# ubc-vision/StableKeypoints

Measured on AMD Instinct MI355X. Metric: images/sec for token-optimization step (SD1.5, 512^2, K=10 kpts), higher is better.
Workload: dtype f32 (fp32 MFMA / VALU throughout; flash attention of the >= 1024-key self-attention layers: 3xbf16 operand split, fp32 accumulate, error <= the fp32 kernel's)

## Files before the change

include/skp.h:

```cpp
#ifndef SKP_H
#define SKP_H

#include <stdint.h>

#ifdef __cplusplus
extern "C" {
#endif

#define SKP_MAX_LAYERS 8
#define SKP_MAX_SUBJECTS 4

#define SKP_E_BADARG (-1)
#define SKP_E_RANGE  (-2)
#define SKP_E_LDS    (-3)

int skp_abi_version(void);

int skp_tune_set(const char* key, int value);
int skp_tune_get(const char* key);

int skp_gemm_nt_f32(const float* A, const float* B, float* C, int M, int N, int K, int Z0, int Z1,
                    int64_t sa0, int64_t sa1, int64_t sam, int64_t sak,
                    int64_t sb0, int64_t sb1, int64_t sbn, int64_t sbk,
                    int64_t sc0, int64_t sc1, int64_t scm, float alpha, void* stream);

int skp_qk_logits_f32(const float* q, const float* k, float* S, int B, int Bk, int H, int T, int s2,
                      int d, float scale, void* stream);

int skp_attn_map_fwd_f32(const float* const* S , const int* s ,
                         int L, int B, int H, int T, int R, float* M, float* lse, void* stream);

int skp_attn_map_fwd_ex_f32(const float* const* S , const int* s , int L, int B, int H,
                            int T, int R, float* M, float* lse_out, const float* lse_in, int ldt,
                            int64_t m_bstride, int mode, void* stream);

int64_t skp_attn_map_bwd_workspace(const int* s , int L, int B, int H, int T, int R);

int skp_attn_map_bwd_f32(const float* const* S , float* const* dS ,
                         const int* s , int L, int B, int H, int T, int R,
                         const float* dM, const float* lse, float* workspace, void* stream);

int skp_attn_map_fwd_wide_f32(const float* const* S , const int* s , int L, int B, int H, int T,
                              int R, float* M, float* lse, const int* tokrow, int n_rows, int ldt, void* stream);
int skp_attn_map_fwd_wide_ok(const int* s , int L, int T, int R);

int skp_attn_map_bwd_col_ok(const int* s , int L, int H, int T, int R, int K);
int64_t skp_attn_map_bwd_col_workspace(const int* s , int L, int B, int H, int T, int R, int K);
int skp_attn_map_bwd_col_f32(const float* const* S , float* const* dS , const int* s , int L,
                             int B, int H, int T, int R, const int64_t* sel, const float* G, int K, const float* lse,
                             void* workspace, int ldt, void* stream);

int64_t skp_attn_map_bwd_sparse_workspace(const int* s , int L, int B, int H, int T, int R, int K);
int skp_attn_map_bwd_sparse_f32(const float* const* S , float* const* dS , const int* s ,
                                int L, int B, int H, int T, int R, const int64_t* sel, const float* G, int K,
                                const float* lse, void* workspace, int ldt, void* stream);

int skp_unwarp_accumulate_f32(const float* M, const float* theta_inv, int n, int K, int R, int S, float* tot, float* num,
                              int finish, void* stream);

int skp_group_norm_coef_f32(const float* x, const float* off, const float* gamma, const float* beta, float* mean, float* rstd,
                            float* coef, const float* bs, int nblk, int pix, float* workspace, int N, int C, int G, int HW,
                            float eps, void* stream);
int skp_conv3x3_f4_gn_ok(int B, int Cin, int Cout, int H, int W);
int skp_conv3x3_f4_gn_f32(const void* x, const void* U, const void* bias, const void* residual, void* y, float* stats,
                          const float* coef, int B, int Cin, int Cout, int H, int W, void* stream);

int skp_conv3x3_f4r_ok(int B, int Cin, int Cout, int H, int W);
int skp_conv3x3_f4r_filter_f32(const void* w, void* R, int Cout, int Cin, int flip_transpose, void* stream);
int64_t skp_conv3x3_f4r_workspace(int B, int Cin, int Cout, int H, int W);
int skp_conv3x3_f4r_f32(const void* x, const void* R, const void* bias, const void* residual, void* y, void* workspace,
                        int B, int Cin, int Cout, int H, int W, void* stream);

int skp_cross_attn_fwd_f32(const float* q, const float* k, const float* v, float* out, float* lse,
                           int B, int Bk, int H, int N, int T, int d, float scale, void* stream);
int64_t skp_cross_attn_bwd_workspace(int B, int H, int N, int T, int d);
int skp_cross_attn_bwd_f32(const float* q, const float* k, const float* v, const float* out,
                           const float* dout, const float* lse, float* dq, float* dk, float* dv,
                           float* workspace, int B, int Bk, int H, int N, int T, int d, float scale,
                           void* stream);

int skp_attn_map_bwd_ex_f32(const float* const* S , float* const* dS , const int* s ,
                            int L, int B, int H, int T, int R, const float* dM, const float* lse,
                            float* workspace, float* dot_io, int ldt, int64_t m_bstride, int mode, void* stream);

int64_t skp_flash_attn_bwd_workspace(int B, int Bk, int H, int N, int Nk, int d);
int skp_flash_attn_fwd_f32(const float* q, const float* k, const float* v, float* out, float* lse,
                           int B, int Bk, int H, int N, int Nk, int d, float scale, void* stream);
int skp_flash_attn_bwd_f32(const float* q, const float* k, const float* v, const float* out, const float* dout,
                           const float* lse, float* dq, float* dk, float* dv, float* workspace,
                           int B, int Bk, int H, int N, int Nk, int d, float scale, void* stream);
int skp_flash_attn_bwd_ld_f32(const float* q, const float* k, const float* v, const float* out, const float* dout,
                              const float* lse, float* dq, float* dk, float* dv, float* workspace,
                              int B, int Bk, int H, int N, int Nk, int d, float scale, int ldg, void* stream);

int skp_flash_attn_fwd_split_ok(int B, int Bk, int H, int N, int Nk, int d);
int64_t skp_flash_attn_fwd_split_workspace(int B, int Bk, int H, int N, int Nk, int d);
int skp_flash_attn_fwd_split_f32(const float* q, const float* k, const float* v, float* out, float* lse, void* workspace,
                                 int B, int Bk, int H, int N, int Nk, int d, float scale, void* stream);
int skp_flash_attn_bwd_split_ok(int B, int Bk, int H, int N, int Nk, int d);
int64_t skp_flash_attn_bwd_split_workspace(int B, int Bk, int H, int N, int Nk, int d);
int skp_flash_attn_bwd_split_f32(const float* q, const float* k, const float* v, const float* out, const float* dout,
                                 const float* lse, float* dq, float* dk, float* dv, void* workspace, int B, int Bk, int H, int N,
                                 int Nk, int d, float scale, void* stream);
int skp_flash_attn_bwd_split_ld_f32(const float* q, const float* k, const float* v, const float* out, const float* dout,
                                    const float* lse, float* dq, float* dk, float* dv, void* workspace, int B, int Bk, int H,
                                    int N, int Nk, int d, float scale, int ldg, void* stream);

int skp_self_attn_fwd_f32(const float* q, const float* k, const float* v, float* out, float* lse,
                          int B, int H, int N, int d, float scale, void* stream);
int skp_self_attn_bwd_f32(const float* q, const float* k, const float* v, const float* out, const float* dout,
                          const float* lse, float* dq, float* dk, float* dv, float* workspace,
                          int B, int H, int N, int d, float scale, void* stream);

int skp_group_norm_fwd_f32(const float* x, const float* off, const float* gamma, const float* beta, float* y,
                           float* mean, float* rstd, float* workspace, int N, int C, int G, int HW, float eps,
                           int silu, void* stream);
int skp_group_norm_onepass_ok(int N, int C, int G, int HW);
int skp_group_norm_bwd_f32(const float* x, const float* off, const float* gamma, const float* beta,
                           const float* dy, const float* mean, const float* rstd, float* dx, float* workspace,
                           int N, int C, int G, int HW, float eps, int silu, void* stream);
int skp_group_norm_bwd_add_f32(const float* x, const float* off, const float* gamma, const float* beta,
                               const float* dy, const float* mean, const float* rstd, float* dx, const float* dadd,
                               float* workspace, int N, int C, int G, int HW, float eps, int silu, void* stream);

int skp_add_bias_residual_f32(const float* a, const float* b, const float* bias, float* out, int N, int C, int HW,
                              void* stream);

int skp_add_layer_norm_ok(int C);
int skp_add_layer_norm_fwd_f32(const float* d, const float* h, const float* gamma, const float* beta, float* x, float* n,
                               float* stat, int64_t rows, int C, float eps, void* stream);
int skp_add_layer_norm_bwd_f32(const float* dn, const float* dskip, const float* x, const float* stat, const float* gamma,
                               float* dx, int64_t rows, int C, void* stream);

int skp_conv3x3_filter_f32(const void* w, void* U, int Cout, int Cin, int flip_transpose, void* stream);
int64_t skp_conv3x3_workspace(int B, int Cin, int Cout, int H, int W, int variant);
int skp_conv3x3_f32(const void* x, const void* U, const void* bias, const void* residual, void* y, void* workspace,
                    int B, int Cin, int Cout, int H, int W, int variant, void* stream);

int skp_conv3x3_f4_filter_f32(const void* w, void* U, int Cout, int Cin, int flip_transpose, void* stream);
int64_t skp_conv3x3_f4_workspace(int B, int Cin, int Cout, int H, int W);
int skp_conv3x3_f4_f32(const void* x, const void* U, const void* bias, const void* residual, void* y, void* workspace,
                       int B, int Cin, int Cout, int H, int W, void* stream);

int skp_conv3x3_f4_stats_blocks(int B, int Cin, int Cout, int H, int W);
int skp_conv3x3_f4_stats_f32(const void* x, const void* U, const void* bias, const void* residual, void* y, float* stats,
                             int B, int Cin, int Cout, int H, int W, void* stream);
int skp_conv3x3_s2_stats_f32(const void* x, const void* U, const void* bias, void* y, float* stats, int B, int Cin, int Cout,
                             int H, int W, int pad, void* stream);
int skp_group_norm_fwd_blocks_f32(const float* x, const float* off, const float* gamma, const float* beta, float* y,
                                  float* mean, float* rstd, const float* bs, int nblk, int pix, int N, int C, int G, int HW,
                                  float eps, int silu, void* stream);

int skp_conv3x3_s2_filter_f32(const void* w, void* U, int Cout, int Cin, void* stream);
int skp_conv3x3_s2_f32(const void* x, const void* U, const void* bias, void* y, int B, int Cin, int Cout, int H, int W,
                       int pad, void* stream);
int64_t skp_conv3x3_s2_workspace(int B, int Cin, int Cout, int H, int W);
int skp_conv3x3_s2_ws_f32(const void* x, const void* U, const void* bias, void* y, void* workspace, int B, int Cin, int Cout,
                          int H, int W, int pad, void* stream);

int skp_conv3x3_small_f32(const void* x, const void* w, const void* bias, void* y, int B, int Cin, int Cout, int H, int W,
                          void* stream);
int skp_conv3x3_small_stats_blocks(int B, int Cin, int Cout, int H, int W);
int skp_conv3x3_small_stats_f32(const void* x, const void* w, const void* bias, void* y, float* stats, int B, int Cin, int Cout,
                                int H, int W, void* stream);

int skp_geglu_fwd_f32(const float* p, float* y, int64_t rows, int inner, void* stream);
int skp_geglu_bwd_f32(const float* p, const float* dy, float* dp, int64_t rows, int inner, void* stream);

int skp_nchw_to_tokens_f32(const float* x, float* y, int B, int C, int HW, void* stream);
int skp_tokens_to_nchw_f32(const float* t, const float* residual, float* y, int B, int C, int HW, void* stream);

int skp_token_stats_f32(const float* M, int T, int R, int num_subjects, float sigma, float eps,
                        int32_t* argmax, float* kl, float* entropy, void* stream);

int skp_select_tokens(const float* kl, const int32_t* argmax_t, int T, int R, int n_cand, int top_k,
                      int64_t* cand, int64_t* sel, void* stream);
int skp_select_tokens_batched(const float* kl, const int32_t* argmax_t, int n, int T, int R, int n_cand, int top_k,
                              int64_t* cand, int64_t* sel, void* stream);

int skp_losses_fwd_f32(const float* M, const float* Mt, const int64_t* sel, int K, int T, int R,
                       const int32_t* argmax, int num_subjects, float sigma,
                       const float* theta_inv , float* partial, float* g_sharp,
                       float* g_eq_a, float* g_eq_b, void* stream);
int skp_losses_fwd_dev_f32(const float* M, const float* Mt, const int64_t* sel, int K, int T, int R,
                           const int32_t* argmax, int num_subjects, float sigma, const float* theta_inv_dev,
                           float* partial, float* g_sharp, float* g_eq_a, float* g_eq_b, void* stream);

int skp_rows_axpy_f32(float* dst, const int64_t* sel, int K, int64_t n, const float* x, const float* a,
                      const float* y, const float* b, void* stream);

#ifdef __cplusplus
}
#endif
#endif
```

stablekeypoints_amd/_native.py:

```python
from __future__ import annotations

import ctypes as C
import os

import torch

_HERE = os.path.dirname(os.path.abspath(__file__))
LIB_PATH = os.environ.get("SKP_LIB_PATH") or os.path.join(_HERE, "csrc", "libskp_hip.so")
ABI_VERSION = 39

_vp, _i, _f, _i64 = C.c_void_p, C.c_int, C.c_float, C.c_int64

SIGNATURES = {
    "skp_abi_version": [],
    "skp_tune_set": [C.c_char_p, _i],
    "skp_tune_get": [C.c_char_p],
    "skp_group_norm_onepass_ok": [_i, _i, _i, _i],
    "skp_gemm_nt_f32": [_vp, _vp, _vp, _i, _i, _i, _i, _i,
                        _i64, _i64, _i64, _i64, _i64, _i64, _i64, _i64, _i64, _i64, _i64, _f, _vp],
    "skp_qk_logits_f32": [_vp, _vp, _vp, _i, _i, _i, _i, _i, _i, _f, _vp],
    "skp_attn_map_fwd_f32": [C.POINTER(_vp), C.POINTER(_i), _i, _i, _i, _i, _i, _vp, _vp, _vp],
    "skp_attn_map_fwd_ex_f32": [C.POINTER(_vp), C.POINTER(_i), _i, _i, _i, _i, _i, _vp, _vp, _vp, _i, _i64, _i, _vp],
    "skp_attn_map_bwd_ex_f32": [C.POINTER(_vp), C.POINTER(_vp), C.POINTER(_i), _i, _i, _i, _i, _i, _vp, _vp, _vp, _vp,
                                _i, _i64, _i, _vp],
    "skp_attn_map_bwd_workspace": [C.POINTER(_i), _i, _i, _i, _i, _i],
    "skp_attn_map_bwd_f32": [C.POINTER(_vp), C.POINTER(_vp), C.POINTER(_i), _i, _i, _i, _i, _i, _vp, _vp, _vp, _vp],
    "skp_group_norm_coef_f32": [_vp, _vp, _vp, _vp, _vp, _vp, _vp, _vp, _i, _i, _vp, _i, _i, _i, _i, _f, _vp],
    "skp_conv3x3_f4_gn_ok": [_i, _i, _i, _i, _i],
    "skp_conv3x3_f4_gn_f32": [_vp, _vp, _vp, _vp, _vp, _vp, _vp, _i, _i, _i, _i, _i, _vp],
    "skp_unwarp_accumulate_f32": [_vp, _vp, _i, _i, _i, _i, _vp, _vp, _i, _vp],
    "skp_attn_map_fwd_wide_f32": [C.POINTER(_vp), C.POINTER(_i), _i, _i, _i, _i, _i, _vp, _vp, _vp, _i, _i, _vp],
    "skp_attn_map_fwd_wide_ok": [C.POINTER(_i), _i, _i, _i],
    "skp_attn_map_bwd_col_ok": [C.POINTER(_i), _i, _i, _i, _i, _i],
    "skp_attn_map_bwd_col_workspace": [C.POINTER(_i), _i, _i, _i, _i, _i, _i],
    "skp_attn_map_bwd_col_f32": [C.POINTER(_vp), C.POINTER(_vp), C.POINTER(_i), _i, _i, _i, _i, _i, _vp, _vp, _i, _vp, _vp,
                                 _i, _vp],
    "skp_attn_map_bwd_sparse_workspace": [C.POINTER(_i), _i, _i, _i, _i, _i, _i],
    "skp_attn_map_bwd_sparse_f32": [C.POINTER(_vp), C.POINTER(_vp), C.POINTER(_i), _i, _i, _i, _i, _i, _vp, _vp, _i, _vp, _vp,
                                    _i, _vp],
    "skp_token_stats_f32": [_vp, _i, _i, _i, _f, _f, _vp, _vp, _vp, _vp],
    "skp_select_tokens": [_vp, _vp, _i, _i, _i, _i, _vp, _vp, _vp],
    "skp_select_tokens_batched": [_vp, _vp, _i, _i, _i, _i, _i, _vp, _vp, _vp],
    "skp_losses_fwd_f32": [_vp, _vp, _vp, _i, _i, _i, _vp, _i, _f, C.POINTER(_f), _vp, _vp, _vp, _vp, _vp],
    "skp_losses_fwd_dev_f32": [_vp, _vp, _vp, _i, _i, _i, _vp, _i, _f, _vp, _vp, _vp, _vp, _vp, _vp],
    "skp_rows_axpy_f32": [_vp, _vp, _i, _i64, _vp, _vp, _vp, _vp, _vp],
    "skp_cross_attn_fwd_f32": [_vp, _vp, _vp, _vp, _vp, _i, _i, _i, _i, _i, _i, _f, _vp],
    "skp_cross_attn_bwd_workspace": [_i, _i, _i, _i, _i],
    "skp_cross_attn_bwd_f32": [_vp, _vp, _vp, _vp, _vp, _vp, _vp, _vp, _vp, _vp, _i, _i, _i, _i, _i, _i, _f, _vp],
    "skp_group_norm_fwd_f32": [_vp, _vp, _vp, _vp, _vp, _vp, _vp, _vp, _i, _i, _i, _i, _f, _i, _vp],
    "skp_group_norm_bwd_f32": [_vp, _vp, _vp, _vp, _vp, _vp, _vp, _vp, _vp, _i, _i, _i, _i, _f, _i, _vp],
    "skp_group_norm_bwd_add_f32": [_vp, _vp, _vp, _vp, _vp, _vp, _vp, _vp, _vp, _vp, _i, _i, _i, _i, _f, _i, _vp],
    "skp_add_bias_residual_f32": [_vp, _vp, _vp, _vp, _i, _i, _i, _vp],
    "skp_add_layer_norm_ok": [_i],
    "skp_add_layer_norm_fwd_f32": [_vp, _vp, _vp, _vp, _vp, _vp, _vp, _i64, _i, _f, _vp],
    "skp_add_layer_norm_bwd_f32": [_vp, _vp, _vp, _vp, _vp, _vp, _i64, _i, _vp],
    "skp_conv3x3_filter_f32": [_vp, _vp, _i, _i, _i, _vp],
    "skp_conv3x3_workspace": [_i, _i, _i, _i, _i, _i],
    "skp_conv3x3_f32": [_vp, _vp, _vp, _vp, _vp, _vp, _i, _i, _i, _i, _i, _i, _vp],
    "skp_conv3x3_f4_filter_f32": [_vp, _vp, _i, _i, _i, _vp],
    "skp_conv3x3_f4_workspace": [_i, _i, _i, _i, _i],
    "skp_conv3x3_f4_f32": [_vp, _vp, _vp, _vp, _vp, _vp, _i, _i, _i, _i, _i, _vp],
    "skp_flash_attn_fwd_split_ok": [_i, _i, _i, _i, _i, _i],
    "skp_flash_attn_fwd_split_workspace": [_i, _i, _i, _i, _i, _i],
    "skp_flash_attn_fwd_split_f32": [_vp, _vp, _vp, _vp, _vp, _vp, _i, _i, _i, _i, _i, _i, C.c_float, _vp],
    "skp_flash_attn_bwd_split_ok": [_i, _i, _i, _i, _i, _i],
    "skp_flash_attn_bwd_split_workspace": [_i, _i, _i, _i, _i, _i],
    "skp_flash_attn_bwd_split_f32": [_vp, _vp, _vp, _vp, _vp, _vp, _vp, _vp, _vp, _vp, _i, _i, _i, _i, _i, _i, _f, _vp],
    "skp_flash_attn_bwd_split_ld_f32": [_vp, _vp, _vp, _vp, _vp, _vp, _vp, _vp, _vp, _vp, _i, _i, _i, _i, _i, _i, _f, _i, _vp],
    "skp_conv3x3_f4r_ok": [_i, _i, _i, _i, _i],
    "skp_conv3x3_f4r_filter_f32": [_vp, _vp, _i, _i, _i, _vp],
    "skp_conv3x3_f4r_workspace": [_i, _i, _i, _i, _i],
    "skp_conv3x3_f4r_f32": [_vp, _vp, _vp, _vp, _vp, _vp, _i, _i, _i, _i, _i, _vp],
    "skp_conv3x3_s2_filter_f32": [_vp, _vp, _i, _i, _vp],
    "skp_conv3x3_s2_f32": [_vp, _vp, _vp, _vp, _i, _i, _i, _i, _i, _i, _vp],
    "skp_conv3x3_s2_workspace": [_i, _i, _i, _i, _i],
    "skp_conv3x3_s2_ws_f32": [_vp, _vp, _vp, _vp, _vp, _i, _i, _i, _i, _i, _i, _vp],
    "skp_conv3x3_small_f32": [_vp, _vp, _vp, _vp, _i, _i, _i, _i, _i, _vp],
    "skp_conv3x3_small_stats_blocks": [_i, _i, _i, _i, _i],
    "skp_conv3x3_small_stats_f32": [_vp, _vp, _vp, _vp, _vp, _i, _i, _i, _i, _i, _vp],
    "skp_conv3x3_f4_stats_blocks": [_i, _i, _i, _i, _i],
    "skp_conv3x3_f4_stats_f32": [_vp, _vp, _vp, _vp, _vp, _vp, _i, _i, _i, _i, _i, _vp],
    "skp_conv3x3_s2_stats_f32": [_vp, _vp, _vp, _vp, _vp, _i, _i, _i, _i, _i, _i, _vp],
    "skp_group_norm_fwd_blocks_f32": [_vp, _vp, _vp, _vp, _vp, _vp, _vp, _vp, _i, _i, _i, _i, _i, _i, _f, _i, _vp],
    "skp_geglu_fwd_f32": [_vp, _vp, _i64, _i, _vp],
    "skp_geglu_bwd_f32": [_vp, _vp, _vp, _i64, _i, _vp],
    "skp_nchw_to_tokens_f32": [_vp, _vp, _i, _i, _i, _vp],
    "skp_tokens_to_nchw_f32": [_vp, _vp, _vp, _i, _i, _i, _vp],
    "skp_flash_attn_fwd_f32": [_vp, _vp, _vp, _vp, _vp, _i, _i, _i, _i, _i, _i, _f, _vp],
    "skp_flash_attn_bwd_workspace": [_i, _i, _i, _i, _i, _i],
    "skp_flash_attn_bwd_f32": [_vp, _vp, _vp, _vp, _vp, _vp, _vp, _vp, _vp, _vp, _i, _i, _i, _i, _i, _i, _f, _vp],
    "skp_flash_attn_bwd_ld_f32": [_vp, _vp, _vp, _vp, _vp, _vp, _vp, _vp, _vp, _vp, _i, _i, _i, _i, _i, _i, _f, _i, _vp],
    "skp_self_attn_fwd_f32": [_vp, _vp, _vp, _vp, _vp, _i, _i, _i, _i, _f, _vp],
    "skp_self_attn_bwd_f32": [_vp, _vp, _vp, _vp, _vp, _vp, _vp, _vp, _vp, _vp, _i, _i, _i, _i, _f, _vp],
}

_ERR = {-1: "SKP_E_BADARG (null pointer / non-positive size)",
        -2: "SKP_E_RANGE (size outside the built kernel range)",
        -3: "SKP_E_LDS (tile exceeds 160 KiB LDS)"}

_lib = None


class NativeLibraryError(RuntimeError):
    pass


def lib():
    global _lib
    if _lib is not None:
        return _lib
    if not os.path.exists(LIB_PATH):
        raise NativeLibraryError(
            f"{LIB_PATH} is missing: build it with `python -c 'import __graft_entry__ as g; g.build()'` "
            "(or `make -C stablekeypoints_amd/csrc`). There is no CPU/eager fallback for the hot path.")
    l = C.CDLL(LIB_PATH)
    for name, argtypes in SIGNATURES.items():
        if not hasattr(l, name):
            raise NativeLibraryError(f"{LIB_PATH} does not export {name}")
        fn = getattr(l, name)
        fn.argtypes = argtypes
        fn.restype = C.c_int64 if name.endswith("_workspace") else C.c_int
    v = l.skp_abi_version()
    if v != ABI_VERSION:
        raise NativeLibraryError(f"ABI mismatch: library {v}, binding {ABI_VERSION}")
    _lib = l
    return l


LAB_PATH = os.environ.get("SKP_LAB_PATH") or os.path.join(os.path.dirname(_HERE), "tools", "csrc", "libskp_lab.so")
LAB_SIGNATURES = {
    "skp_probe_mfma_f32": [_i, _i, _vp, _vp, _vp],
}
_lab = None


def lab():
    global _lab
    if _lab is None:
        if not os.path.exists(LAB_PATH):
            raise NativeLibraryError(f"{LAB_PATH} is missing: `make -C tools/csrc` (measurement aids, not the product library)")
        l = C.CDLL(LAB_PATH)
        for name, argtypes in LAB_SIGNATURES.items():
            fn = getattr(l, name)
            fn.argtypes, fn.restype = argtypes, C.c_int
        _lab = l
    return _lab


def check(rc: int, what: str):
    if rc == 0:
        return
    if rc < 0:
        raise RuntimeError(f"{what}: {_ERR.get(rc, rc)}")
    raise RuntimeError(f"{what}: HIP launch failed with hipError_t={rc}")


def ptr_array(ptrs):
    arr = (C.c_void_p * len(ptrs))(*[C.c_void_p(int(p)) for p in ptrs])
    return C.cast(arr, C.POINTER(C.c_void_p)), arr


def int_array(vals):
    arr = (C.c_int * len(vals))(*[int(v) for v in vals])
    return C.cast(arr, C.POINTER(C.c_int)), arr


def float_array(vals):
    arr = (C.c_float * len(vals))(*[float(v) for v in vals])
    return C.cast(arr, C.POINTER(C.c_float)), arr


def tune(key: str, value: int) -> None:
    check(lib().skp_tune_set(key.encode(), int(value)), f"skp_tune_set({key})")
```

stablekeypoints_amd/csrc/skp_conv_wino4.hip:

```cpp
#include <algorithm>
#include <type_traits>
#include "skp_common.h"
#include "skp_wino4_common.h"
#include <stdlib.h>

namespace {

__global__ void skp_wino4_filter_kernel(const float* __restrict__ w, float* __restrict__ U, int Cout, int Cin, int flip_t) {
    const int idx = blockIdx.x * blockDim.x + threadIdx.x;
    if (idx >= Cout * Cin) return;
    const int co = idx / Cin, ci = idx - co * Cin;
    float g[3][3];
    if (!flip_t) {
        const float* p = w + ((size_t)co * Cin + ci) * 9;
#pragma unroll
        for (int a = 0; a < 3; ++a)
#pragma unroll
            for (int b = 0; b < 3; ++b) g[a][b] = p[a * 3 + b];
    } else {
        const float* p = w + ((size_t)ci * Cout + co) * 9;
#pragma unroll
        for (int a = 0; a < 3; ++a)
#pragma unroll
            for (int b = 0; b < 3; ++b) g[a][b] = p[(2 - a) * 3 + (2 - b)];
// ... 113 lines not shown
#pragma unroll
    for (int tb = 0; tb < 2; ++tb) {
        const int tg = tile0 + tb * 16 + i16;
        t_ok[tb] = tg < a.nTiles;
        const int tgc = t_ok[tb] ? tg : 0;
        const int b = tgc / a.tilesPerImg, rem = tgc - b * a.tilesPerImg;
        const int ty = rem / a.tilesX, tx = rem - ty * a.tilesX;
        o_base[tb] = ((b * a.Cout) * a.H + 4 * ty) * a.W + 4 * tx;
    }

#pragma unroll
    for (int i = 0; i < 6; ++i) { load_row(cin_begin, 0, i); load_row(cin_begin, 1, i); }
#pragma unroll
    for (int k = 0; k < 3; ++k) { col_pass(0, k); col_pass(1, k); }
#pragma unroll
    for (int i = 0; i < 6; ++i) row_pass_store(0, i);
    f32x4 ua[W4_RING];
#pragma unroll
    for (int q = 0; q < W4_RING - 1; ++q) ua[q] = skp_buf_load_f32x4(urs, uvo, (cin_begin >> 4) * u_c16 + q * u_p, 0);
    __syncthreads();

    auto run_stage = [&](int s, auto mode_c) {
        constexpr int MODE = decltype(mode_c)::value;
        const f32x4* vb = vst + (s & 1) * W4_STAGE_F4 + kq * 32 + i16;
        const int ub = ((cin_begin >> 4) + s) * u_c16;
        f32x4 va[3][2];
        va[0][0] = vb[0];
        va[0][1] = vb[16];
        va[1][0] = vb[128];
        va[1][1] = vb[128 + 16];
        w4_unroll([&](auto pc) {
            constexpr int p = decltype(pc)::value;
            {
                constexpr int D = W4_RING - 1;
                constexpr int q = p + D;
                if (MODE == 0 || q < 36) {
                    const int uo = q < 36 ? ub + q * u_p : ub + u_c16 + (q - 36) * u_p;
                    ua[q % W4_RING] = skp_buf_load_f32x4(urs, uvo, uo, 0);
                }
            }
            if (MODE == 0) {
                if (p < 6) {
                    load_row(cin_begin + (s + 1) * 16, 0, p);
                    load_row(cin_begin + (s + 1) * 16, 1, p);
                } else if (p >= 24 && p < 30) {
                    col_pass((p - 24) & 1, (p - 24) >> 1);
                } else if (p >= 30) {
                    row_pass_store((s + 1) & 1, p - 30);
                }
            }
            if (p + 2 < 36) {
                va[(p + 2) % 3][0] = vb[(p + 2) * 128];
                va[(p + 2) % 3][1] = vb[(p + 2) * 128 + 16];
            }
            w4_unroll([&](auto mc) {
                constexpr int m = decltype(mc)::value;
                w4c_mfma<p, 0>(accv, ua[p % W4_RING][m], va[p % 3][0][m]);
                w4c_mfma<p, 1>(accv, ua[p % W4_RING][m], va[p % 3][1][m]);
            }, std::make_integer_sequence<int, 4>{});
            __builtin_amdgcn_sched_barrier(0);
        }, std::make_integer_sequence<int, 36>{});
    };
    for (int s = 0; s + 1 < nsteps; ++s) {
        run_stage(s, std::integral_constant<int, 0>{});
        __syncthreads();
    }
    run_stage(nsteps - 1, std::integral_constant<int, 1>{});
    if (STATS) __syncthreads();

    const i32x4 yrs = skp_make_rsrc(a.y + zsplit * a.y_split_stride, a.y_bytes);
    const i32x4 rrs = skp_make_rsrc(a.res, a.res ? a.y_bytes : 0u);
    const i32x4 brs = skp_make_rsrc(a.bias, a.bias ? (unsigned)a.Cout * 4u : 0u);
    f32x4 rr[4][2][4];
    float bvs[4];
    auto load_res = [&](int r) {
        const int co = n0 + 4 * kq + r;
#pragma unroll
        for (int tb = 0; tb < 2; ++tb) {
            const bool ok = t_ok[tb] && co < a.Cout;
            const int vo = (o_base[tb] + co * HW) * 4;
#pragma unroll
            for (int oy = 0; oy < 4; ++oy) rr[r][tb][oy] = skp_buf_load_f32x4(rrs, ok ? vo + oy * a.W * 4 : SKP_OOB, 0, 0);
        }
    };
#pragma unroll
    for (int r = 0; r < 4; ++r) {
        const int co = n0 + 4 * kq + r;
        bvs[r] = skp_buf_load_f32(brs, co < a.Cout ? co * 4 : SKP_OOB, 0, 0);
    }
    load_res(0);
    load_res(1);
    asm volatile("s_nop 15\n\ts_nop 15" ::: "memory");
    __builtin_amdgcn_sched_barrier(0);
    w4_unroll([&](auto rc) {
        constexpr int r = decltype(rc)::value;
        const int co = n0 + 4 * kq + r;
        const float bv = bvs[r];
        if (r + 2 < 4) load_res(r + 2);
        w4_unroll([&](auto tbc) {
            constexpr int tb = decltype(tbc)::value;
            const bool ok = t_ok[tb] && co < a.Cout;
            const int vo = (o_base[tb] + co * HW) * 4;
            float t[6][4];
            w4_unroll([&](auto ic) {
                constexpr int i = decltype(ic)::value;
                float m[6];
                w4_unroll([&](auto jc) { constexpr int j = decltype(jc)::value; m[j] = w4c_acc<i * 6 + j, tb, r>(accv); },
                          std::make_integer_sequence<int, 6>{});
                w4_out1d(m, t[i]);
            }, std::make_integer_sequence<int, 6>{});
#pragma unroll
            for (int ox = 0; ox < 4; ++ox) {
                float m[6], yv[4];
#pragma unroll
                for (int i = 0; i < 6; ++i) m[i] = t[i][ox];
                w4_out1d(m, yv);
#pragma unroll
                for (int oy = 0; oy < 4; ++oy) rr[r][tb][oy][ox] += yv[oy] + bv;
            }
#pragma unroll
            for (int oy = 0; oy < 4; ++oy) skp_buf_store_f32x4(rr[r][tb][oy], yrs, ok ? vo + oy * a.W * 4 : SKP_OOB, 0, 0);
            if (STATS) w4_park_stats((f32x2*)vst, wave * 8 + r * 2 + tb, lane, rr[r][tb], ok);
            __builtin_amdgcn_sched_barrier(0);
        }, std::make_integer_sequence<int, 2>{});
    }, std::make_integer_sequence<int, 4>{});
    if (STATS) {
        __syncthreads();
        if (tid < 128) {
            const int wv = tid >> 5, tb = (tid >> 4) & 1, lc = tid & 15;
            w4_store_stats(a, (const f32x2*)vst, wv * 8 + (lc & 3) * 2 + tb, lc >> 2, tile0 + tb * 16, (cg * 4 + wv) * 16 + lc);
        }
    }
}

__global__ void skp_wino4r_filter_kernel(const float* __restrict__ w, float* __restrict__ R, int Cout, int Cin, int flip_t) {
    const int idx = blockIdx.x * blockDim.x + threadIdx.x;
    if (idx >= Cout * Cin) return;
    const int co = idx / Cin, ci = idx - co * Cin;
    const int c16 = ci >> 4, kq = (ci >> 2) & 3, m = ci & 3, cb = co >> 4, i16 = co & 15, CB = Cout >> 4;
    float* dst = R + ((size_t)(c16 * CB + cb) * 9 * 64 + kq * 16 + i16) * 4 + m;
#pragma unroll
    for (int t = 0; t < 9; ++t) {
        const float v = flip_t ? w[((size_t)ci * Cout + co) * 9 + (8 - t)] : w[((size_t)co * Cin + ci) * 9 + t];
        dst[t * 256] = v;
    }
}

__global__ __launch_bounds__(256) void skp_wino4r_input_kernel(const float* __restrict__ x, float* __restrict__ Vg, int B, int Cin, int H,
                                                               int W, int tilesX, int tilesPerImg, int nTiles, int vpad) {
    const int idx = blockIdx.x * 256 + threadIdx.x;
    const int m = idx & 3, rest = idx >> 2;
    const int tg = rest % vpad, q4 = rest / vpad;
    if (q4 >= (Cin >> 2)) return;
    const bool tv = tg < nTiles;
    const int tgc = tv ? tg : 0;
    const int b = tgc / tilesPerImg, rem = tgc - b * tilesPerImg;
    const int ty = rem / tilesX, tx = rem - ty * tilesX;
    const float dsc[6] = {0.25f, -1.f / 6, -1.f / 6, 1.f / 24, 1.f / 24, 1.f};
    const float* xc = x + ((size_t)b * Cin + q4 * 4 + m) * H * W;
    float d[6][6];
#pragma unroll
    for (int i = 0; i < 6; ++i) {
        const int r = 4 * ty - 1 + i;
        const bool rv = tv && r >= 0 && r < H;
        const float* row = xc + r * W + 4 * tx;
        const f32x4 mid = rv ? *(const f32x4*)row : f32x4{0.f, 0.f, 0.f, 0.f};
        d[i][0] = (rv && tx > 0) ? row[-1] : 0.f;
        d[i][1] = mid[0]; d[i][2] = mid[1]; d[i][3] = mid[2]; d[i][4] = mid[3];
        d[i][5] = (rv && tx + 1 < tilesX) ? row[4] : 0.f;
    }
#pragma unroll
    for (int j = 0; j < 6; ++j) {
        float v[6], t[6];
#pragma unroll
        for (int i = 0; i < 6; ++i) v[i] = d[i][j];
        w4_in1d(v, t);
#pragma unroll
        for (int i = 0; i < 6; ++i) d[i][j] = t[i];
    }
    const int c16 = q4 >> 2, kq = q4 & 3;
    float* dst = Vg + (((size_t)c16 * 36 * 4 + kq) * vpad + tg) * 4 + m;
#pragma unroll
    for (int i = 0; i < 6; ++i) {
        float t[6];
        w4_in1d(d[i], t);
#pragma unroll
        for (int j = 0; j < 6; ++j) dst[(size_t)(i * 6 + j) * 16 * vpad] = t[j] * (dsc[i] * dsc[j]);
    }
}

#ifdef W4R_STAMPS
__device__ unsigned long long w4r_stamps[2][64];
#define W4R_STAMP(k) do { if (tid == 0 && (blockIdx.x == 0 || blockIdx.x == 100) && (k) < 64) w4r_stamps[blockIdx.x ? 1 : 0][k] = __builtin_readcyclecounter(); } while (0)
#else
#define W4R_STAMP(k) do { } while (0)
#endif
template <bool PART, int NTB = 2>
__global__ __launch_bounds__(256, 1) void skp_wino4r_conv_kernel(Wino4Args a) {
    extern __shared__ f32x4 vst[];
    const int tid = threadIdx.x, lane = tid & 63, wave = __builtin_amdgcn_readfirstlane(tid >> 6);
    const int i16 = lane & 15, kq = lane >> 4;
    int tblock, cg, zsplit;
    if (!w4_work(a, blockIdx.x + blockIdx.z * gridDim.x, tblock, cg, zsplit)) return;
    W4R_STAMP(0);
    const int tile0 = tblock * 32;
    const int n0 = (cg * 4 + wave) * 16;
    const int HW = a.H * a.W;
    const int nsteps = min(a.steps, a.total_steps - zsplit * a.steps);
    const int c16_0 = zsplit * a.steps;
    const i32x4 vrs = skp_make_rsrc(a.x, a.x_bytes);
    const i32x4 wrs = skp_make_rsrc(a.U, a.u_bytes);

    const int v_vo = ((tid >> 5) * a.vpad + tile0 + (tid & 31)) * 16;
    const int v_row8 = a.vpad * 128;
    auto load_v = [&](int c16, int buf, int r) {
        skp_buf_load_lds(vrs, (skp_lds_ptr)(vst + buf * W4_STAGE_F4 + r * 256 + wave * 64), 16, v_vo, c16 * 18 * v_row8 + r * v_row8, 0, 0);
    };
    const int CB = a.Cout >> 4;
    const int w_cb = ((cg * 4 + wave) * 9) * 1024;
    const int w_c16 = CB * 9 * 1024;
    f32x4 g[9], gn[9];
    auto load_g = [&](f32x4 (&dst)[9], int c16) {
#pragma unroll
        for (int t = 0; t < 9; ++t) dst[t] = skp_buf_load_f32x4(wrs, lane * 16, c16 * w_c16 + w_cb + t * 1024, 0);
    };
    f32x4 ut[3];
    auto u_piece = [&](const f32x4 (&gg)[9], int i, int piece, f32x4 (&u)[6]) {
        if (piece < 3) {
            const int b = piece;
            const f32x4 g0 = gg[b], g1 = gg[3 + b], g2 = gg[6 + b];
            ut[b] = i == 0 ? g0 : i == 5 ? g2 : i == 1 ? (g0 + g2) + g1 : i == 2 ? (g0 + g2) - g1
                  : i == 3 ? (g0 + 4.f * g2) + 2.f * g1 : (g0 + 4.f * g2) - 2.f * g1;
        } else if (piece == 3) {
            const f32x4 s2 = ut[0] + ut[2];
            u[0] = ut[0]; u[5] = ut[2];
            u[1] = s2 + ut[1]; u[2] = s2 - ut[1];
        } else if (piece == 4) {
            const f32x4 e = ut[0] + 4.f * ut[2];
            u[3] = e + 2.f * ut[1];
        } else {
            const f32x4 e = ut[0] + 4.f * ut[2];
            u[4] = e - 2.f * ut[1];
        }
    };
    auto u_row = [&](const f32x4 (&gg)[9], int i, f32x4 (&u)[6]) {
#pragma unroll
        for (int k = 0; k < 6; ++k) u_piece(gg, i, k, u);
    };

    w4_unroll([&](auto rc) { asm volatile("v_accvgpr_write_b32 a[%0], 0" : : "n"(decltype(rc)::value) : W4_AGPR_CLOBBERS); },
              std::make_integer_sequence<int, 256>{});
    f32x4 accv[4][2];
#pragma unroll
    for (int p = 0; p < 4; ++p)
#pragma unroll
        for (int tb = 0; tb < 2; ++tb) accv[p][tb] = f32x4{0.f, 0.f, 0.f, 0.f};

    int o_base[2];
    bool t_ok[2];
#pragma unroll
    for (int tb = 0; tb < 2; ++tb) {
        const int tg = tile0 + tb * 16 + i16;
        t_ok[tb] = tg < a.nTiles;
        const int tgc = t_ok[tb] ? tg : 0;
        const int b = tgc / a.tilesPerImg, rem = tgc - b * a.tilesPerImg;
        const int ty = rem / a.tilesX, tx = rem - ty * a.tilesX;
        o_base[tb] = ((b * a.Cout) * a.H + 4 * ty) * a.W + 4 * tx;
    }

#pragma unroll
    for (int r = 0; r < 18; ++r) load_v(c16_0, 0, r);
    load_g(g, c16_0);
    f32x4 ur[2][6];
    u_row(g, 0, ur[0]);
    asm volatile("s_waitcnt vmcnt(0)" ::: "memory");
    __syncthreads();
    W4R_STAMP(1);

    for (int s = 0; s < nsteps; ++s) {
        const f32x4* vb = vst + (s & 1) * W4_STAGE_F4 + kq * 32 + i16;
        const int c16n = c16_0 + min(s + 1, nsteps - 1);
        f32x4 va[3][2];
        va[0][0] = vb[0];
        va[1][0] = vb[128];
        if (NTB == 2) { va[0][1] = vb[16]; va[1][1] = vb[128 + 16]; }
        w4_unroll([&](auto pc) {
            constexpr int p = decltype(pc)::value, i = p / 6, j = p - 6 * i;
            if (p == 0) load_g(gn, c16n);
            else if (p <= 18) load_v(c16n, (s + 1) & 1, p - 1);
            if (i < 5) u_piece(g, i + 1, j, ur[(i + 1) & 1]);
            if (p + 2 < 36) {
                va[(p + 2) % 3][0] = vb[(p + 2) * 128];
                if (NTB == 2) va[(p + 2) % 3][1] = vb[(p + 2) * 128 + 16];
            }
            w4_unroll([&](auto mc) {
                constexpr int m = decltype(mc)::value;
                w4c_mfma<p, 0>(accv, ur[i & 1][j][m], va[p % 3][0][m]);
                if constexpr (NTB == 2) w4c_mfma<p, 1>(accv, ur[i & 1][j][m], va[p % 3][1][m]);
            }, std::make_integer_sequence<int, 4>{});
            __builtin_amdgcn_sched_barrier(0);
        }, std::make_integer_sequence<int, 36>{});
#pragma unroll
        for (int t = 0; t < 9; ++t) g[t] = gn[t];
        u_row(g, 0, ur[0]);
        asm volatile("s_waitcnt vmcnt(0)" ::: "memory");
        __syncthreads();
        W4R_STAMP(2 + s);
    }

    asm volatile("s_nop 15\n\ts_nop 15" ::: "memory");
    __builtin_amdgcn_sched_barrier(0);
    const i32x4 yrs = skp_make_rsrc(a.y + zsplit * a.y_split_stride, a.y_bytes);
    if (PART) {
        w4_unroll([&](auto rc) {
            constexpr int r = decltype(rc)::value;
            const int co = n0 + 4 * kq + r;
            w4_unroll([&](auto tbc) {
                constexpr int tb = decltype(tbc)::value;
                const bool ok = t_ok[tb] && co < a.Cout;
                const int vo = (o_base[tb] + co * HW) * 4;
                float t[6][4];
                w4_unroll([&](auto ic) {
                    constexpr int i = decltype(ic)::value;
                    float m[6];
                    w4_unroll([&](auto jc) { constexpr int j = decltype(jc)::value; m[j] = w4c_acc<i * 6 + j, tb, r>(accv); },
                              std::make_integer_sequence<int, 6>{});
                    w4_out1d(m, t[i]);
                }, std::make_integer_sequence<int, 6>{});
                f32x4 o[4];
#pragma unroll
                for (int ox = 0; ox < 4; ++ox) {
                    float m[6], yv[4];
#pragma unroll
                    for (int i = 0; i < 6; ++i) m[i] = t[i][ox];
                    w4_out1d(m, yv);
#pragma unroll
                    for (int oy = 0; oy < 4; ++oy) o[oy][ox] = yv[oy];
                }
#pragma unroll
                for (int oy = 0; oy < 4; ++oy) skp_buf_store_f32x4(o[oy], yrs, ok ? vo + oy * a.W * 4 : SKP_OOB, 0, 0);
                __builtin_amdgcn_sched_barrier(0);
// ... 297 lines not shown
                w4_unroll([&](auto jc) { constexpr int j = decltype(jc)::value; m[j] = w4c_acc<i * 6 + j, cb, r>(accv); },
                          std::make_integer_sequence<int, 6>{});
                w4_out1d(m, t[i]);
            }, std::make_integer_sequence<int, 6>{});
#pragma unroll
            for (int ox = 0; ox < 4; ++ox) {
                float m[6], yv[4];
#pragma unroll
                for (int i = 0; i < 6; ++i) m[i] = t[i][ox];
                w4_out1d(m, yv);
#pragma unroll
                for (int oy = 0; oy < 4; ++oy) rr[e][oy][ox] += yv[oy] + bv;
            }
#pragma unroll
            for (int oy = 0; oy < 4; ++oy) skp_buf_store_f32x4(rr[e][oy], yrs, ok ? vo + oy * a.W * 4 : SKP_OOB, 0, 0);
            if (STATS) w4_park_stats(sst, wave * 8 + e, lane, rr[e], ok);
            __builtin_amdgcn_sched_barrier(0);
        }, std::make_integer_sequence<int, 8>{});
        if (STATS) {
            __syncthreads();
            if (tid < 128) {
                const int wv = tid >> 5, lc = tid & 31;
                w4_store_stats(a, sst, wv * 8 + ((lc >> 4) << 2) + (lc & 3), (lc >> 2) & 3, tile0, (cg * 4 + wv) * 32 + lc);
            }
        }
        if (!has_next) break;
        bpar = (bpar + nsteps) & 1;
        wid = wnext; tblock = tb_n; cg = cg_n; zsplit = z_n;
    }
}

static bool wino4_use_c128(int Cout, int tiles) {
    return tiles >= 128 && (Cout % 128 == 0 || (Cout > 128 && Cout % 128 >= 64));
}

static Wino4Grid wino4_grid(int Cout, int tiles, int S) {
    Wino4Grid g;
    const bool c128 = wino4_use_c128(Cout, tiles);
    g.ntb = c128 ? (tiles + 15) / 16 : (tiles + 31) / 32;
    g.ncg = c128 ? (Cout + 127) / 128 : (Cout + 63) / 64;
    g.tb_per_xcd = g.ntb >= (c128 ? 64 : 32) ? (g.ntb + 7) / 8 : 0;
    if (g.tb_per_xcd) {
        g.gx = 8u * g.tb_per_xcd * g.ncg;
        g.rounds = (int)((g.gx * (unsigned)S + 255) / 256);
    } else {
        const int upx = (g.ncg * S + 7) / 8;
        g.gx = 8u * upx * g.ntb;
        g.rounds = (upx * g.ntb + 31) / 32;
    }
    return g;
}

int wino4_plan(int B, int Cin, int Cout, int H, int W) {
    if (B <= 0 || Cin <= 0 || Cout <= 0 || H <= 0 || W <= 0) return 0;
    if ((Cin % 16) || (Cout % 16) || (H % 4) || (W % 4)) return 0;
    const int tiles = B * (H / 4) * (W / 4);
    const bool c128 = wino4_use_c128(Cout, tiles);
    const int nsteps = Cin / 16;
    const double out_bytes = (double)B * Cout * H * W * 4;
    if (const int S = skp_tune(SKP_TUNE_WINO_SPLIT)) {
        if (S >= 1 && S <= 16 && (S - 1) * ((nsteps + S - 1) / S) < nsteps) return S;
    }
    int best = 1;
    double best_cost = 1e30;
    const bool ragged_c128 = c128 && (Cout % 128) != 0;
    const double stage_us = c128 ? (ragged_c128 ? 4.8 : 3.9) : 5.6;
    for (int S = 1; S <= 16; ++S) {
        const int per = (nsteps + S - 1) / S;
        if ((S - 1) * per >= nsteps) continue;
        const Wino4Grid g = wino4_grid(Cout, tiles, S);
        double cost = g.rounds * (per + 2.0) * stage_us;
        if (S > 1) cost += 6.0 + (S + 1) * out_bytes / 8.0e6;
        if (cost < best_cost * (S > 1 ? (ragged_c128 ? 0.95 : 0.92) : 1.0)) { best_cost = cost; best = S; }
    }
    return best;
}

static Wino4Grid wino4r_grid(int Cout, int tiles, int S) {
    Wino4Grid g;
    g.ntb = (tiles + 31) / 32;
    g.ncg = Cout / 64;
    g.tb_per_xcd = g.ntb >= 32 ? (g.ntb + 7) / 8 : 0;
    if (g.tb_per_xcd) {
        g.gx = 8u * g.tb_per_xcd * g.ncg;
        g.rounds = (int)((g.gx * (unsigned)S + 255) / 256);
    } else {
        const int upx = (g.ncg * S + 7) / 8;
        g.gx = 8u * upx * g.ntb;
        g.rounds = (upx * g.ntb + 31) / 32;
    }
    return g;
}
static int wino4r_max_tiles() { return skp_tune(SKP_TUNE_WINO_RAW_MAX_TILES); }
static bool wino4r_layout_ok(int B, int Cin, int Cout, int H, int W) {
    if (B <= 0 || Cin <= 0 || Cout <= 0 || H <= 0 || W <= 0) return false;
    if ((Cin % 16) || (Cout % 64) || (H % 4) || (W % 4)) return false;
    const long long tiles = (long long)B * (H / 4) * (W / 4);
    const long long vpad = (tiles + 31) / 32 * 32;
    return 36ll * Cin * vpad * 4 < 0x7fffffffll && 9ll * Cin * Cout * 4 < 0x7fffffffll && (long long)B * Cout * H * W * 4 < 0x7fffffffll;
}
static bool wino4r_shape_ok(int B, int Cin, int Cout, int H, int W) {
    if (!wino4r_layout_ok(B, Cin, Cout, H, W)) return false;
    const long long tiles = (long long)B * (H / 4) * (W / 4);
    if (wino4r_max_tiles() > 0) return tiles <= wino4r_max_tiles() && Cin >= 256;
    if (Cin >= 1280 && Cout >= 1280) return tiles <= 1536;
    return tiles <= 512 && (Cin >= 1920 || Cout >= 1920) && Cin >= 640 && Cout >= 640;
}
constexpr double W4R_STAGE1_US = 2.7;
static int wino4r_plan(int B, int Cin, int Cout, int H, int W) {
    const int tiles = B * (H / 4) * (W / 4);
    const int nsteps = Cin / 16;
    const double out_bytes = (double)B * Cout * H * W * 4;
    if (const int S = skp_tune(SKP_TUNE_WINO_SPLIT)) {
        if (S >= 1 && S <= 16 && (S - 1) * ((nsteps + S - 1) / S) < nsteps) return S;
    }
    int best = 1;
    double best_cost = 1e30;
    const double stage_us = tiles <= 16 ? W4R_STAGE1_US : 4.8, over = tiles <= 16 ? 2.0 : 2.5;
    for (int S = 1; S <= 16; ++S) {
        const int per = (nsteps + S - 1) / S;
        if ((S - 1) * per >= nsteps) continue;
        const Wino4Grid g = wino4r_grid(Cout, tiles, S);
        double cost = g.rounds * (per + over) * stage_us;
        if (S > 1) cost += 6.0 + (S + 1) * out_bytes / 8.0e6;
        if (cost < best_cost * (S > 1 ? 0.97 : 1.0)) { best_cost = cost; best = S; }
    }
    return best;
}

}

extern "C" int skp_conv3x3_f4_filter_f32(const void* w, void* U, int Cout, int Cin, int flip_transpose, void* stream) {
    if (!w || !U || Cout <= 0 || Cin <= 0) return SKP_E_BADARG;
    if (Cin & 15) return SKP_E_RANGE;
    const int n = Cout * Cin;
    hipLaunchKernelGGL(skp_wino4_filter_kernel, dim3((n + 255) / 256), dim3(256), 0, (hipStream_t)stream, (const float*)w,
                       (float*)U, Cout, Cin, flip_transpose);
    return skp_launch_status();
}

extern "C" int64_t skp_conv3x3_f4_workspace(int B, int Cin, int Cout, int H, int W) {
    const int S = wino4_plan(B, Cin, Cout, H, W);
    return S > 1 ? (int64_t)S * B * Cout * H * W * (int64_t)sizeof(float) : 0;
}

extern "C" int skp_conv3x3_f4_stats_blocks(int B, int Cin, int Cout, int H, int W) {
    const int S = wino4_plan(B, Cin, Cout, H, W);
    if (S != 1) return 0;
    const int tpi = (H / 4) * (W / 4);
    return (tpi % 32 == 0) ? tpi / 16 : 0;
}

static int wino4_run(const void* x, const void* U, const void* bias, const void* residual, void* y, void* workspace, float* stats,
                     int B, int Cin, int Cout, int H, int W, void* stream, const float* gncoef = nullptr);

extern "C" int skp_conv3x3_f4_gn_ok(int B, int Cin, int Cout, int H, int W) {
    if (wino4_plan(B, Cin, Cout, H, W) != 1) return 0;
    const int tiles = B * (H / 4) * (W / 4);
    const int max_cout = skp_tune(SKP_TUNE_GN_FOLD_MAX_COUT) ? skp_tune(SKP_TUNE_GN_FOLD_MAX_COUT) : 512;
    return (wino4_use_c128(Cout, tiles) && Cout <= max_cout) ? 1 : 0;
}

extern "C" int skp_conv3x3_f4_gn_f32(const void* x, const void* U, const void* bias, const void* residual, void* y,
                                     float* stats, const float* coef, int B, int Cin, int Cout, int H, int W, void* stream) {
    if (!coef) return SKP_E_BADARG;
    if (!skp_conv3x3_f4_gn_ok(B, Cin, Cout, H, W)) return SKP_E_RANGE;
    if (stats && skp_conv3x3_f4_stats_blocks(B, Cin, Cout, H, W) == 0) return SKP_E_RANGE;
    return wino4_run(x, U, bias, residual, y, nullptr, stats, B, Cin, Cout, H, W, stream, coef);
}

extern "C" int skp_conv3x3_f4_f32(const void* x, const void* U, const void* bias, const void* residual, void* y,
                                  void* workspace, int B, int Cin, int Cout, int H, int W, void* stream) {
    return wino4_run(x, U, bias, residual, y, workspace, nullptr, B, Cin, Cout, H, W, stream);
}

extern "C" int skp_conv3x3_f4_stats_f32(const void* x, const void* U, const void* bias, const void* residual, void* y,
                                        float* stats, int B, int Cin, int Cout, int H, int W, void* stream) {
    if (!stats || skp_conv3x3_f4_stats_blocks(B, Cin, Cout, H, W) == 0) return SKP_E_RANGE;
    return wino4_run(x, U, bias, residual, y, nullptr, stats, B, Cin, Cout, H, W, stream);
}

static int wino4_run(const void* x, const void* U, const void* bias, const void* residual, void* y, void* workspace, float* stats,
                     int B, int Cin, int Cout, int H, int W, void* stream, const float* gncoef) {
    if (!x || !U || !y) return SKP_E_BADARG;
    int S = wino4_plan(B, Cin, Cout, H, W);
    if (S == 0) return (B <= 0 || Cin <= 0 || Cout <= 0 || H <= 0 || W <= 0) ? SKP_E_BADARG : SKP_E_RANGE;
    if (!workspace) S = 1;
    const unsigned long long xb = (unsigned long long)B * Cin * H * W * 4, ub = (unsigned long long)36 * Cin * Cout * 4,
                             yb = (unsigned long long)B * Cout * H * W * 4;
    if (xb >= 0x80000000ull || ub >= 0x80000000ull || yb >= 0x80000000ull) return SKP_E_RANGE;
    Wino4Args a;
    a.x = (const float*)x; a.U = (const float*)U;
    a.B = B; a.Cin = Cin; a.Cout = Cout; a.H = H; a.W = W;
    a.tilesX = W / 4;
    a.tilesPerImg = a.tilesX * (H / 4);
    a.nTiles = B * a.tilesPerImg;
    a.x_bytes = (unsigned)xb; a.u_bytes = (unsigned)ub; a.y_bytes = (unsigned)yb;
    a.total_steps = Cin / 16;
    a.steps = (a.total_steps + S - 1) / S;
    a.splits = S;
    const size_t out_elems = (size_t)B * Cout * H * W;
    a.y_split_stride = out_elems;
    a.y = S > 1 ? (float*)workspace : (float*)y;
    a.bias = S > 1 ? nullptr : (const float*)bias;
    a.res = S > 1 ? nullptr : (const float*)residual;
    a.stats = S > 1 ? nullptr : stats;
    a.sblk = a.tilesPerImg / 16;
    a.gncoef = gncoef;
    hipStream_t st = (hipStream_t)stream;
    const size_t lds = (size_t)2 * W4_STAGE_F4 * sizeof(f32x4), lds_c = (size_t)2 * W4C_STAGE_F4 * sizeof(f32x4) + 32 * 64 * sizeof(f32x2);
    static bool attr_set = false;
    if (!attr_set) {
        hipError_t e = hipFuncSetAttribute((const void*)skp_wino4_conv_kernel<false>, hipFuncAttributeMaxDynamicSharedMemorySize, (int)lds);
        if (e != hipSuccess) return (int)e;
        e = hipFuncSetAttribute((const void*)skp_wino4_conv_kernel<true>, hipFuncAttributeMaxDynamicSharedMemorySize, (int)lds);
        if (e != hipSuccess) return (int)e;
        e = hipFuncSetAttribute((const void*)skp_wino4_conv_c128_kernel<false>, hipFuncAttributeMaxDynamicSharedMemorySize, (int)lds_c);
        if (e != hipSuccess) return (int)e;
        e = hipFuncSetAttribute((const void*)skp_wino4_conv_c128_kernel<true>, hipFuncAttributeMaxDynamicSharedMemorySize, (int)lds_c);
        if (e != hipSuccess) return (int)e;
        e = hipFuncSetAttribute((const void*)skp_wino4_conv_c128_kernel<true, true>, hipFuncAttributeMaxDynamicSharedMemorySize, (int)lds_c);
        if (e != hipSuccess) return (int)e;
        e = hipFuncSetAttribute((const void*)skp_wino4_conv_c128_kernel<false, true>, hipFuncAttributeMaxDynamicSharedMemorySize, (int)lds_c);
        if (e != hipSuccess) return (int)e;
        attr_set = true;
    }
    const bool c128 = wino4_use_c128(Cout, a.nTiles);
    const Wino4Grid g = wino4_grid(Cout, a.nTiles, S);
    a.ntb = g.ntb; a.ncg = g.ncg; a.tb_per_xcd = g.tb_per_xcd;
    a.gx = (int)g.gx;
    a.vtotal = g.tb_per_xcd ? (int)g.gx * S : (int)g.gx;
    static const int persist = [] {
        int dev = 0, ncu = 0;
        if (hipGetDevice(&dev) != hipSuccess || hipDeviceGetAttribute(&ncu, hipDeviceAttributeMultiprocessorCount, dev) != hipSuccess) ncu = 256;
        return ncu;
    }();
    const dim3 grid = c128 ? dim3((unsigned)(persist >= 8 ? std::min(a.vtotal, persist & ~7) : a.vtotal), 1, 1)
                           : (g.tb_per_xcd ? dim3(g.gx, 1, S) : dim3(g.gx, 1, 1));
    if (c128) {
        if (gncoef) {
            if (a.stats) hipLaunchKernelGGL((skp_wino4_conv_c128_kernel<true, true>), grid, dim3(256), lds_c, st, a);
            else hipLaunchKernelGGL((skp_wino4_conv_c128_kernel<false, true>), grid, dim3(256), lds_c, st, a);
        } else if (a.stats) hipLaunchKernelGGL((skp_wino4_conv_c128_kernel<true>), grid, dim3(256), lds_c, st, a);
        else hipLaunchKernelGGL((skp_wino4_conv_c128_kernel<false>), grid, dim3(256), lds_c, st, a);
    } else if (gncoef) {
        return SKP_E_RANGE;
    } else {
        if (a.stats) hipLaunchKernelGGL(skp_wino4_conv_kernel<true>, grid, dim3(256), lds, st, a);
        else hipLaunchKernelGGL(skp_wino4_conv_kernel<false>, grid, dim3(256), lds, st, a);
    }
    int rc = skp_launch_status();
    if (rc || S == 1) return rc;
    const size_t n4 = out_elems / 4;
    hipLaunchKernelGGL(skp_wino4_reduce_kernel, dim3((unsigned)((n4 + 255) / 256)), dim3(256), 0, st, (const float*)workspace,
                       (const float*)bias, (const float*)residual, (float*)y, n4, out_elems, S, (H * W) / 4, Cout);
    return skp_launch_status();
}

extern "C" int skp_conv3x3_f4r_ok(int B, int Cin, int Cout, int H, int W) {
    return wino4r_shape_ok(B, Cin, Cout, H, W) ? 1 : 0;
}

extern "C" int skp_conv3x3_f4r_filter_f32(const void* w, void* R, int Cout, int Cin, int flip_transpose, void* stream) {
    if (!w || !R || Cout <= 0 || Cin <= 0) return SKP_E_BADARG;
    if ((Cin & 15) || (Cout & 15)) return SKP_E_RANGE;
    const int n = Cout * Cin;
    hipLaunchKernelGGL(skp_wino4r_filter_kernel, dim3((n + 255) / 256), dim3(256), 0, (hipStream_t)stream, (const float*)w,
                       (float*)R, Cout, Cin, flip_transpose);
    return skp_launch_status();
}

extern "C" int64_t skp_conv3x3_f4r_workspace(int B, int Cin, int Cout, int H, int W) {
    if (!wino4r_layout_ok(B, Cin, Cout, H, W)) return 0;
    const int64_t tiles = (int64_t)B * (H / 4) * (W / 4), vpad = (tiles + 31) / 32 * 32;
    const int S = wino4r_plan(B, Cin, Cout, H, W);
    return 36 * (int64_t)Cin * vpad * 4 + (S > 1 ? (int64_t)S * B * Cout * H * W * 4 : 0);
}

extern "C" int skp_conv3x3_f4r_f32(const void* x, const void* R, const void* bias, const void* residual, void* y, void* workspace,
                                   int B, int Cin, int Cout, int H, int W, void* stream) {
    if (!x || !R || !y || !workspace) return SKP_E_BADARG;
    if (!wino4r_layout_ok(B, Cin, Cout, H, W)) return (B <= 0 || Cin <= 0 || Cout <= 0 || H <= 0 || W <= 0) ? SKP_E_BADARG : SKP_E_RANGE;
    const int S = wino4r_plan(B, Cin, Cout, H, W);
    Wino4Args a;
    a.B = B; a.Cin = Cin; a.Cout = Cout; a.H = H; a.W = W;
    a.tilesX = W / 4;
    a.tilesPerImg = a.tilesX * (H / 4);
    a.nTiles = B * a.tilesPerImg;
    a.vpad = (a.nTiles + 31) / 32 * 32;
    const size_t v_elems = (size_t)36 * Cin * a.vpad;
    float* Vg = (float*)workspace;
    float* part = Vg + v_elems;
    a.x = Vg; a.U = (const float*)R;
    a.x_bytes = (unsigned)(v_elems * 4); a.u_bytes = (unsigned)((size_t)9 * Cin * Cout * 4);
    const size_t out_elems = (size_t)B * Cout * H * W;
    a.y_bytes = (unsigned)(out_elems * 4);
    a.total_steps = Cin / 16;
    a.steps = (a.total_steps + S - 1) / S;
    a.splits = S;
    a.y_split_stride = out_elems;
    a.y = S > 1 ? part : (float*)y;
    a.bias = S > 1 ? nullptr : (const float*)bias;
    a.res = S > 1 ? nullptr : (const float*)residual;
    a.stats = nullptr; a.sblk = 0; a.gncoef = nullptr;
    hipStream_t st = (hipStream_t)stream;
    const size_t lds = (size_t)2 * W4_STAGE_F4 * sizeof(f32x4);
    static bool attr_set = false;
    if (!attr_set) {
        hipError_t e = hipFuncSetAttribute((const void*)skp_wino4r_conv_kernel<true>, hipFuncAttributeMaxDynamicSharedMemorySize, (int)lds);
        if (e != hipSuccess) return (int)e;
        e = hipFuncSetAttribute((const void*)skp_wino4r_conv_kernel<false>, hipFuncAttributeMaxDynamicSharedMemorySize, (int)lds);
        if (e != hipSuccess) return (int)e;
        e = hipFuncSetAttribute((const void*)skp_wino4r_conv_kernel<true, 1>, hipFuncAttributeMaxDynamicSharedMemorySize, (int)lds);
        if (e != hipSuccess) return (int)e;
        e = hipFuncSetAttribute((const void*)skp_wino4r_conv_kernel<false, 1>, hipFuncAttributeMaxDynamicSharedMemorySize, (int)lds);
        if (e != hipSuccess) return (int)e;
        attr_set = true;
    }
    const Wino4Grid g = wino4r_grid(Cout, a.nTiles, S);
    a.ntb = g.ntb; a.ncg = g.ncg; a.tb_per_xcd = g.tb_per_xcd;
    a.gx = (int)g.gx;
    a.vtotal = g.tb_per_xcd ? (int)g.gx * S : (int)g.gx;
    const int nin = a.vpad * Cin;
    hipLaunchKernelGGL(skp_wino4r_input_kernel, dim3((unsigned)((nin + 255) / 256)), dim3(256), 0, st, (const float*)x, Vg, B, Cin, H, W,
                       a.tilesX, a.tilesPerImg, a.nTiles, a.vpad);
    const dim3 grid = g.tb_per_xcd ? dim3(g.gx, 1, S) : dim3(g.gx, 1, 1);
    if (a.nTiles <= 16) {
        if (S > 1) hipLaunchKernelGGL((skp_wino4r_conv_kernel<true, 1>), grid, dim3(256), lds, st, a);
        else hipLaunchKernelGGL((skp_wino4r_conv_kernel<false, 1>), grid, dim3(256), lds, st, a);
    } else if (S > 1) hipLaunchKernelGGL(skp_wino4r_conv_kernel<true>, grid, dim3(256), lds, st, a);
    else hipLaunchKernelGGL(skp_wino4r_conv_kernel<false>, grid, dim3(256), lds, st, a);
    int rc = skp_launch_status();
    if (rc || S == 1) return rc;
    const size_t n4 = out_elems / 4;
    hipLaunchKernelGGL(skp_wino4_reduce_kernel, dim3((unsigned)((n4 + 255) / 256)), dim3(256), 0, st, (const float*)part,
                       (const float*)bias, (const float*)residual, (float*)y, n4, out_elems, S, (H * W) / 4, Cout);
    return skp_launch_status();
}

#ifdef W4R_STAMPS
extern "C" int skp_w4r_read_stamps(unsigned long long* out) {
    return (int)hipMemcpyFromSymbol(out, HIP_SYMBOL(w4r_stamps), sizeof(unsigned long long) * 128);
}
#endif
```

stablekeypoints_amd/csrc/skp_group_norm.hip:

```cpp
#include "skp_common.h"
#include <stdlib.h>

struct GNArgs {
    const float* x; const float* off; const float* gamma; const float* beta;
    int N, C, G, HW, nsplit, silu;
    float eps;
    long L;
};

__global__ __launch_bounds__(256) void skp_gn_stats_kernel(GNArgs a, float* __restrict__ partial) {
    __shared__ float red[4];
    const int row = blockIdx.y, split = blockIdx.x, tid = threadIdx.x;
    const int n = row / a.G, g = row - n * a.G, Cg = a.C / a.G;
    const float* xr = a.x + (size_t)row * a.L;
    const float* offr = a.off ? a.off + (size_t)n * a.C + g * Cg : nullptr;
    const long q4 = a.L / 4;
    const long per = (q4 + a.nsplit - 1) / a.nsplit;
    const long lo = split * per, hi = (lo + per < q4) ? lo + per : q4;
    const float K = xr[0] + (offr ? offr[0] : 0.f);
    float s1 = 0.f, s2 = 0.f;
    const int hw4 = a.HW / 4;
    for (long i = lo + tid; i < hi; i += 256) {
        f32x4 v = *(const f32x4*)(xr + i * 4);
        if (offr) v += offr[i / hw4];
        v -= K;
        s1 += (v[0] + v[1]) + (v[2] + v[3]);
        s2 += (v[0] * v[0] + v[1] * v[1]) + (v[2] * v[2] + v[3] * v[3]);
    }
    s1 = skp_block_sum_256(s1, red);
    s2 = skp_block_sum_256(s2, red);
    if (tid == 0) {
        float* p = partial + ((size_t)row * a.nsplit + split) * 3;
        p[0] = K; p[1] = s1; p[2] = s2;
    }
}

__device__ __forceinline__ void skp_gn_finalize(const float* partial, int row, int nsplit, long L, float eps,
                                                float& mean, float& rstd) {
    double s1 = 0.0, s2 = 0.0;
    const float K = partial[(size_t)row * nsplit * 3];
    for (int i = 0; i < nsplit; ++i) {
        const float* p = partial + ((size_t)row * nsplit + i) * 3;
        s1 += (double)p[1]; s2 += (double)p[2];
    }
    const double m = s1 / (double)L;
    double var = s2 / (double)L - m * m;
    var = var < 0.0 ? 0.0 : var;
    mean = (float)((double)K + m);
    rstd = (float)(1.0 / sqrt(var + (double)eps));
}

__global__ __launch_bounds__(256) void skp_gn_from_blocks_kernel(GNArgs a, const float* __restrict__ bs, int nblk, int pix,
                                                                 float* __restrict__ mean_out, float* __restrict__ rstd_out) {
    __shared__ double red[4];
    __shared__ double gmean;
    const int row = blockIdx.x, tid = threadIdx.x;
    const int n = row / a.G, g = row - n * a.G, Cg = a.C / a.G;
    auto block_sum = [&](double v) {
#pragma unroll
        for (int o = 32; o > 0; o >>= 1) v += __shfl_xor(v, o, 64);
        __syncthreads();
        if ((tid & 63) == 0) red[tid >> 6] = v;
        __syncthreads();
        return (red[0] + red[1]) + (red[2] + red[3]);
    };
    double s1 = 0.0;
    for (int e = tid; e < Cg * nblk; e += 256) {
        const int cl = e / nblk, blk = e - cl * nblk, c = g * Cg + cl;
        const double o = a.off ? (double)a.off[(size_t)n * a.C + c] : 0.0;
        s1 += (double)bs[(((size_t)n * a.C + c) * nblk + blk) * 2] + o;
    }
    const double m = block_sum(s1) / (double)(Cg * nblk);
    if (tid == 0) gmean = m;
    __syncthreads();
    double m2 = 0.0;
    for (int e = tid; e < Cg * nblk; e += 256) {
        const int cl = e / nblk, blk = e - cl * nblk, c = g * Cg + cl;
        const float* p = bs + (((size_t)n * a.C + c) * nblk + blk) * 2;
        const double o = a.off ? (double)a.off[(size_t)n * a.C + c] : 0.0;
        const double d = (double)p[0] + o - gmean;
        m2 += (double)p[1] + (double)pix * d * d;
    }
    const double t2 = block_sum(m2);
    if (tid == 0) {
        double var = t2 / (double)a.L;
        var = var < 0.0 ? 0.0 : var;
        mean_out[row] = (float)gmean;
        rstd_out[row] = (float)(1.0 / sqrt(var + (double)a.eps));
    }
}

__global__ __launch_bounds__(256) void skp_gn_apply_kernel(GNArgs a, const float* __restrict__ partial,
                                                           float* __restrict__ y, float* __restrict__ mean_out,
                                                           float* __restrict__ rstd_out) {
    const int row = blockIdx.y, tid = threadIdx.x;
    const int n = row / a.G, g = row - n * a.G, Cg = a.C / a.G;
    float mean, rstd;
    if (partial) {
        skp_gn_finalize(partial, row, a.nsplit, a.L, a.eps, mean, rstd);
        if (blockIdx.x == 0 && tid == 0) { mean_out[row] = mean; rstd_out[row] = rstd; }
    } else {
        mean = mean_out[row]; rstd = rstd_out[row];
    }
    const float* xr = a.x + (size_t)row * a.L;
    float* yr = y + (size_t)row * a.L;
    const int hw4 = a.HW / 4;
    const long q4 = a.L / 4;
    for (long i = (long)blockIdx.x * 256 + tid; i < q4; i += (long)gridDim.x * 256) {
        const int cl = (int)(i / hw4), c = g * Cg + cl;
        const float sc = rstd * a.gamma[c];
        const float sh = a.beta[c] + ((a.off ? a.off[(size_t)n * a.C + c] : 0.f) - mean) * sc;
        f32x4 v = *(const f32x4*)(xr + i * 4);
        v = v * sc + sh;
        if (a.silu) {
#pragma unroll
            for (int e = 0; e < 4; ++e) v[e] = v[e] / (1.0f + __expf(-v[e]));
        }
        *(f32x4*)(yr + i * 4) = v;
    }
}

__global__ __launch_bounds__(256) void skp_gn_bwd_stats_kernel(GNArgs a, const float* __restrict__ dy,
                                                               const float* __restrict__ mean_in,
                                                               const float* __restrict__ rstd_in,
                                                               float* __restrict__ partial) {
    __shared__ float red[4];
    const int row = blockIdx.y, split = blockIdx.x, tid = threadIdx.x;
    const int n = row / a.G, g = row - n * a.G, Cg = a.C / a.G;
    const float mean = mean_in[row], rstd = rstd_in[row];
    const float* xr = a.x + (size_t)row * a.L;
    const float* dr = dy + (size_t)row * a.L;
    const int hw4 = a.HW / 4;
    const long q4 = a.L / 4;
    const long per = (q4 + a.nsplit - 1) / a.nsplit;
    const long lo = split * per, hi = (lo + per < q4) ? lo + per : q4;
    float s1 = 0.f, s2 = 0.f;
    for (long i = lo + tid; i < hi; i += 256) {
        const int c = g * Cg + (int)(i / hw4);
        const float gam = a.gamma[c], bet = a.beta[c];
        const float o = a.off ? a.off[(size_t)n * a.C + c] : 0.f;
        const f32x4 xv = *(const f32x4*)(xr + i * 4);
        const f32x4 dv = *(const f32x4*)(dr + i * 4);
#pragma unroll
        for (int e = 0; e < 4; ++e) {
            const float xh = (xv[e] + o - mean) * rstd;
            float gz = dv[e];
            if (a.silu) {
                const float z = xh * gam + bet;
                const float sg = 1.0f / (1.0f + __expf(-z));
                gz *= sg * (1.0f + z * (1.0f - sg));
            }
            gz *= gam;
            s1 += gz; s2 += gz * xh;
        }
    }
    s1 = skp_block_sum_256(s1, red);
    s2 = skp_block_sum_256(s2, red);
    if (tid == 0) {
        float* p = partial + ((size_t)row * a.nsplit + split) * 2;
        p[0] = s1; p[1] = s2;
    }
}

__global__ __launch_bounds__(256) void skp_gn_bwd_apply_kernel(GNArgs a, const float* __restrict__ dy,
                                                               const float* __restrict__ mean_in,
                                                               const float* __restrict__ rstd_in,
                                                               const float* __restrict__ partial,
                                                               float* __restrict__ dx, const float* __restrict__ dadd) {
    const int row = blockIdx.y, tid = threadIdx.x;
    const int n = row / a.G, g = row - n * a.G, Cg = a.C / a.G;
    const float mean = mean_in[row], rstd = rstd_in[row];
    double t1 = 0.0, t2 = 0.0;
    for (int i = 0; i < a.nsplit; ++i) {
        const float* p = partial + ((size_t)row * a.nsplit + i) * 2;
        t1 += (double)p[0]; t2 += (double)p[1];
    }
    const float m1 = (float)(t1 / (double)a.L), m2 = (float)(t2 / (double)a.L);
    const float* xr = a.x + (size_t)row * a.L;
    const float* dr = dy + (size_t)row * a.L;
    float* dxr = dx + (size_t)row * a.L;
    const int hw4 = a.HW / 4;
    const long q4 = a.L / 4;
    for (long i = (long)blockIdx.x * 256 + tid; i < q4; i += (long)gridDim.x * 256) {
        const int c = g * Cg + (int)(i / hw4);
        const float gam = a.gamma[c], bet = a.beta[c];
        const float o = a.off ? a.off[(size_t)n * a.C + c] : 0.f;
        const f32x4 xv = *(const f32x4*)(xr + i * 4);
        const f32x4 dv = *(const f32x4*)(dr + i * 4);
        f32x4 r;
#pragma unroll
        for (int e = 0; e < 4; ++e) {
            const float xh = (xv[e] + o - mean) * rstd;
            float gz = dv[e];
            if (a.silu) {
                const float z = xh * gam + bet;
                const float sg = 1.0f / (1.0f + __expf(-z));
                gz *= sg * (1.0f + z * (1.0f - sg));
            }
            gz *= gam;
            r[e] = rstd * (gz - m1 - xh * m2);
        }
        if (dadd) r += *(const f32x4*)(dadd + (size_t)row * a.L + i * 4);
        *(f32x4*)(dxr + i * 4) = r;
    }
}

__device__ __forceinline__ float skp_block_sum_1024(float v, float* red) {
#pragma unroll
    for (int o = 32; o > 0; o >>= 1) v += __shfl_xor(v, o, 64);
    __syncthreads();
    if ((threadIdx.x & 63) == 0) red[threadIdx.x >> 6] = v;
    __syncthreads();
    float t = 0.f;
#pragma unroll
    for (int w = 0; w < 16; ++w) t += red[w];
    return t;
}

template <int VPT>
__global__ __launch_bounds__(1024) void skp_gn_onepass_fwd_kernel(GNArgs a, float* __restrict__ y, float* __restrict__ mean_out,
                                                                  float* __restrict__ rstd_out) {
    __shared__ float red[16];
    const int row = blockIdx.x, tid = threadIdx.x;
    const int n = row / a.G, g = row - n * a.G, Cg = a.C / a.G;
    const float* xr = a.x + (size_t)row * a.L;
    float* yr = y + (size_t)row * a.L;
    const int hw4 = a.HW / 4, q4 = (int)(a.L / 4);
    f32x4 v[VPT];
    float s = 0.f;
#pragma unroll
    for (int j = 0; j < VPT; ++j) {
        const int i = tid + 1024 * j;
        v[j] = f32x4{0.f, 0.f, 0.f, 0.f};
        if (i < q4) {
            v[j] = *(const f32x4*)(xr + (size_t)i * 4);
            if (a.off) v[j] += a.off[(size_t)n * a.C + g * Cg + i / hw4];
            s += (v[j][0] + v[j][1]) + (v[j][2] + v[j][3]);
        }
    }
    const float mean = skp_block_sum_1024(s, red) / (float)a.L;
    float s2 = 0.f;
#pragma unroll
    for (int j = 0; j < VPT; ++j)
        if (tid + 1024 * j < q4) {
            const f32x4 d = v[j] - mean;
            s2 += (d[0] * d[0] + d[1] * d[1]) + (d[2] * d[2] + d[3] * d[3]);
        }
    const float var = skp_block_sum_1024(s2, red) / (float)a.L;
    const float rstd = 1.0f / sqrtf(var + a.eps);
    if (tid == 0) { mean_out[row] = mean; rstd_out[row] = rstd; }
#pragma unroll
    for (int j = 0; j < VPT; ++j) {
        const int i = tid + 1024 * j;
        if (i < q4) {
            const int c = g * Cg + i / hw4;
            const float sc = rstd * a.gamma[c];
            const float sh = a.beta[c] - mean * sc;
            f32x4 r = v[j] * sc + sh;
            if (a.silu) {
#pragma unroll
                for (int e = 0; e < 4; ++e) r[e] = r[e] / (1.0f + __expf(-r[e]));
            }
            *(f32x4*)(yr + (size_t)i * 4) = r;
        }
    }
}

template <int VPT>
__global__ __launch_bounds__(1024) void skp_gn_onepass_bwd_kernel(GNArgs a, const float* __restrict__ dy, const float* __restrict__ mean_in,
                                                                  const float* __restrict__ rstd_in, float* __restrict__ dx,
                                                                  const float* __restrict__ dadd) {
    __shared__ float red[16];
    const int row = blockIdx.x, tid = threadIdx.x;
    const int n = row / a.G, g = row - n * a.G, Cg = a.C / a.G;
    const float mean = mean_in[row], rstd = rstd_in[row];
    const float* xr = a.x + (size_t)row * a.L;
    const float* dr = dy + (size_t)row * a.L;
    float* dxr = dx + (size_t)row * a.L;
    const int hw4 = a.HW / 4, q4 = (int)(a.L / 4);
    f32x4 xh[VPT], gz[VPT];
    float s1 = 0.f, s2 = 0.f;
#pragma unroll
    for (int j = 0; j < VPT; ++j) {
        const int i = tid + 1024 * j;
        xh[j] = f32x4{0.f, 0.f, 0.f, 0.f};
        gz[j] = f32x4{0.f, 0.f, 0.f, 0.f};
        if (i < q4) {
            const int c = g * Cg + i / hw4;
            const float gam = a.gamma[c], bet = a.beta[c];
            const float o = a.off ? a.off[(size_t)n * a.C + c] : 0.f;
            const f32x4 xv = *(const f32x4*)(xr + (size_t)i * 4);
            const f32x4 dv = *(const f32x4*)(dr + (size_t)i * 4);
#pragma unroll
            for (int e = 0; e < 4; ++e) {
                const float h = (xv[e] + o - mean) * rstd;
                float t = dv[e];
                if (a.silu) {
                    const float z = h * gam + bet;
                    const float sg = 1.0f / (1.0f + __expf(-z));
                    t *= sg * (1.0f + z * (1.0f - sg));
                }
                t *= gam;
                xh[j][e] = h; gz[j][e] = t;
                s1 += t; s2 += t * h;
            }
        }
    }
    const float m1 = skp_block_sum_1024(s1, red) / (float)a.L;
    const float m2 = skp_block_sum_1024(s2, red) / (float)a.L;
#pragma unroll
    for (int j = 0; j < VPT; ++j) {
        const int i = tid + 1024 * j;
        if (i < q4) {
            f32x4 r = (gz[j] - m1 - xh[j] * m2) * rstd;
            if (dadd) r += *(const f32x4*)(dadd + (size_t)row * a.L + (size_t)i * 4);
            *(f32x4*)(dxr + (size_t)i * 4) = r;
        }
    }
}

static int gn_onepass_vpt(const GNArgs& a, bool backward) {
    const long q4 = a.L / 4, need = (q4 + 1023) / 1024;
    const int fsizes[] = {1, 2, 4, 10, 16}, bsizes[] = {1, 2, 4, 8, 10};
    for (int k = 0; k < 5; ++k) {
        const int v = backward ? bsizes[k] : fsizes[k];
        if (need <= v) return v;
    }
    return 0;
}

static int gn_onepass_fwd(const GNArgs& a, float* y, float* mean, float* rstd, hipStream_t st) {
    const dim3 grid(a.N * a.G), block(1024);
    switch (gn_onepass_vpt(a, false)) {
        case 1: hipLaunchKernelGGL(skp_gn_onepass_fwd_kernel<1>, grid, block, 0, st, a, y, mean, rstd); break;
        case 2: hipLaunchKernelGGL(skp_gn_onepass_fwd_kernel<2>, grid, block, 0, st, a, y, mean, rstd); break;
        case 4: hipLaunchKernelGGL(skp_gn_onepass_fwd_kernel<4>, grid, block, 0, st, a, y, mean, rstd); break;
        case 10: hipLaunchKernelGGL(skp_gn_onepass_fwd_kernel<10>, grid, block, 0, st, a, y, mean, rstd); break;
        case 16: hipLaunchKernelGGL(skp_gn_onepass_fwd_kernel<16>, grid, block, 0, st, a, y, mean, rstd); break;
        default: return -100;
    }
    return skp_launch_status();
}

static int gn_onepass_bwd(const GNArgs& a, const float* dy, const float* mean, const float* rstd, float* dx, const float* dadd,
                          hipStream_t st) {
    const dim3 grid(a.N * a.G), block(1024);
    switch (gn_onepass_vpt(a, true)) {
        case 1: hipLaunchKernelGGL(skp_gn_onepass_bwd_kernel<1>, grid, block, 0, st, a, dy, mean, rstd, dx, dadd); break;
        case 2: hipLaunchKernelGGL(skp_gn_onepass_bwd_kernel<2>, grid, block, 0, st, a, dy, mean, rstd, dx, dadd); break;
        case 4: hipLaunchKernelGGL(skp_gn_onepass_bwd_kernel<4>, grid, block, 0, st, a, dy, mean, rstd, dx, dadd); break;
        case 8: hipLaunchKernelGGL(skp_gn_onepass_bwd_kernel<8>, grid, block, 0, st, a, dy, mean, rstd, dx, dadd); break;
        case 10: hipLaunchKernelGGL(skp_gn_onepass_bwd_kernel<10>, grid, block, 0, st, a, dy, mean, rstd, dx, dadd); break;
        default: return -100;
    }
    return skp_launch_status();
}

static int gn_fill(GNArgs& a, const float* x, const float* off, const float* gamma, const float* beta, int N, int C,
                   int G, int HW, float eps, int silu) {
    if (!x || !gamma || !beta || N <= 0 || C <= 0 || G <= 0 || HW <= 0) return SKP_E_BADARG;
    if (C % G || HW % 4 || (long)N * G > 65535) return SKP_E_RANGE;
    a.x = x; a.off = off; a.gamma = gamma; a.beta = beta;
    a.N = N; a.C = C; a.G = G; a.HW = HW; a.eps = eps; a.silu = silu;
    a.L = (long)(C / G) * HW;
    long rows = (long)N * G, want = (2048 + rows - 1) / rows, cap = a.L / 4096;
    if (cap < 1) cap = 1;
    a.nsplit = (int)(want < cap ? want : cap);
    if (a.nsplit < 1) a.nsplit = 1;
    if (a.nsplit > 64) a.nsplit = 64;
    return 0;
}

extern "C" int skp_group_norm_nsplit(int N, int C, int G, int HW) {
    GNArgs a{};
    static const float dummy = 0.f;
    int rc = gn_fill(a, &dummy, nullptr, &dummy, &dummy, N, C, G, HW, 1e-5f, 0);
    return rc ? rc : a.nsplit;
}

extern "C" int skp_group_norm_onepass_ok(int N, int C, int G, int HW) {
    if (N <= 0 || C <= 0 || G <= 0 || HW <= 0 || C % G || (HW & 3)) return 0;
    GNArgs a{};
    a.N = N; a.C = C; a.G = G; a.HW = HW; a.L = (long)(C / G) * HW;
    return gn_onepass_vpt(a, false) ? 1 : 0;
}

extern "C" int skp_group_norm_fwd_f32(const float* x, const float* off, const float* gamma, const float* beta,
                                      float* y, float* mean, float* rstd, float* workspace, int N, int C, int G,
                                      int HW, float eps, int silu, void* stream) {
    GNArgs a{};
    int rc = gn_fill(a, x, off, gamma, beta, N, C, G, HW, eps, silu);
    if (rc) return rc;
    if (!y || !mean || !rstd || !workspace) return SKP_E_BADARG;
    hipStream_t st = (hipStream_t)stream;
    if (gn_onepass_vpt(a, false)) return gn_onepass_fwd(a, y, mean, rstd, st);
    hipLaunchKernelGGL(skp_gn_stats_kernel, dim3(a.nsplit, N * G), dim3(256), 0, st, a, workspace);
    rc = skp_launch_status();
    if (rc) return rc;
    long blocks = (a.L / 4 + 256 * 8 - 1) / (256 * 8);
    if (blocks < 1) blocks = 1;
    if (blocks > 64) blocks = 64;
    hipLaunchKernelGGL(skp_gn_apply_kernel, dim3((unsigned)blocks, N * G), dim3(256), 0, st, a,
                       (const float*)workspace, y, mean, rstd);
    return skp_launch_status();
}

extern "C" int skp_group_norm_fwd_blocks_f32(const float* x, const float* off, const float* gamma, const float* beta,
                                             float* y, float* mean, float* rstd, const float* bs, int nblk, int pix, int N, int C,
                                             int G, int HW, float eps, int silu, void* stream) {
    GNArgs a{};
    int rc = gn_fill(a, x, off, gamma, beta, N, C, G, HW, eps, silu);
    if (rc) return rc;
    if (!y || !mean || !rstd || !bs || nblk <= 0 || pix <= 0) return SKP_E_BADARG;
    if ((long)nblk * pix != HW) return SKP_E_RANGE;
    hipStream_t st = (hipStream_t)stream;
    if (gn_onepass_vpt(a, false)) return gn_onepass_fwd(a, y, mean, rstd, st);
    hipLaunchKernelGGL(skp_gn_from_blocks_kernel, dim3(N * G), dim3(256), 0, st, a, bs, nblk, pix, mean, rstd);
    rc = skp_launch_status();
    if (rc) return rc;
    long blocks = (a.L / 4 + 256 * 8 - 1) / (256 * 8);
    if (blocks < 1) blocks = 1;
    if (blocks > 64) blocks = 64;
    hipLaunchKernelGGL(skp_gn_apply_kernel, dim3((unsigned)blocks, N * G), dim3(256), 0, st, a, (const float*)nullptr, y, mean,
                       rstd);
    return skp_launch_status();
}

__global__ __launch_bounds__(256) void skp_gn_coef_kernel(GNArgs a, const float* __restrict__ partial, float* __restrict__ mean_io,
                                                          float* __restrict__ rstd_io, float* __restrict__ coef) {
    const int i = blockIdx.x * 256 + threadIdx.x;
    if (i >= a.N * a.C) return;
    const int n = i / a.C, c = i - n * a.C, Cg = a.C / a.G, row = n * a.G + c / Cg;
    float mean, rstd;
    if (partial) {
        skp_gn_finalize(partial, row, a.nsplit, a.L, a.eps, mean, rstd);
        if (c % Cg == 0) { mean_io[row] = mean; rstd_io[row] = rstd; }
    } else {
        mean = mean_io[row]; rstd = rstd_io[row];
    }
    const float sc = rstd * a.gamma[c];
    coef[2 * i] = sc;
    coef[2 * i + 1] = a.beta[c] + ((a.off ? a.off[i] : 0.f) - mean) * sc;
}

extern "C" int skp_group_norm_coef_f32(const float* x, const float* off, const float* gamma, const float* beta, float* mean,
                                       float* rstd, float* coef, const float* bs, int nblk, int pix, float* workspace, int N,
                                       int C, int G, int HW, float eps, void* stream) {
    GNArgs a;
    int rc = gn_fill(a, x ? x : gamma, off, gamma, beta, N, C, G, HW, eps, 0);
    if (rc) return rc;
    if (!mean || !rstd || !coef) return SKP_E_BADARG;
    hipStream_t st = (hipStream_t)stream;
    const unsigned nb = (unsigned)((N * C + 255) / 256);
    if (bs) {
        if (nblk <= 0 || pix <= 0) return SKP_E_BADARG;
        if ((long)nblk * pix != HW) return SKP_E_RANGE;
        hipLaunchKernelGGL(skp_gn_from_blocks_kernel, dim3(N * G), dim3(256), 0, st, a, bs, nblk, pix, mean, rstd);
        hipLaunchKernelGGL(skp_gn_coef_kernel, dim3(nb), dim3(256), 0, st, a, (const float*)nullptr, mean, rstd, coef);
    } else {
        if (!x || !workspace) return SKP_E_BADARG;
        hipLaunchKernelGGL(skp_gn_stats_kernel, dim3(a.nsplit, N * G), dim3(256), 0, st, a, workspace);
        hipLaunchKernelGGL(skp_gn_coef_kernel, dim3(nb), dim3(256), 0, st, a, (const float*)workspace, mean, rstd, coef);
    }
    return skp_launch_status();
}

static int gn_bwd_run(const float* x, const float* off, const float* gamma, const float* beta, const float* dy, const float* mean,
                      const float* rstd, float* dx, const float* dadd, float* workspace, int N, int C, int G, int HW, float eps,
                      int silu, void* stream);

extern "C" int skp_group_norm_bwd_f32(const float* x, const float* off, const float* gamma, const float* beta,
                                      const float* dy, const float* mean, const float* rstd, float* dx,
                                      float* workspace, int N, int C, int G, int HW, float eps, int silu,
                                      void* stream) {
    return gn_bwd_run(x, off, gamma, beta, dy, mean, rstd, dx, nullptr, workspace, N, C, G, HW, eps, silu, stream);
}

extern "C" int skp_group_norm_bwd_add_f32(const float* x, const float* off, const float* gamma, const float* beta,
                                          const float* dy, const float* mean, const float* rstd, float* dx, const float* dadd,
                                          float* workspace, int N, int C, int G, int HW, float eps, int silu, void* stream) {
    if (!dadd) return SKP_E_BADARG;
    return gn_bwd_run(x, off, gamma, beta, dy, mean, rstd, dx, dadd, workspace, N, C, G, HW, eps, silu, stream);
}

static int gn_bwd_run(const float* x, const float* off, const float* gamma, const float* beta, const float* dy, const float* mean,
                      const float* rstd, float* dx, const float* dadd, float* workspace, int N, int C, int G, int HW, float eps,
                      int silu, void* stream) {
    GNArgs a{};
    int rc = gn_fill(a, x, off, gamma, beta, N, C, G, HW, eps, silu);
    if (rc) return rc;
    if (!dy || !mean || !rstd || !dx || !workspace) return SKP_E_BADARG;
    hipStream_t st = (hipStream_t)stream;
    if (gn_onepass_vpt(a, true)) return gn_onepass_bwd(a, dy, mean, rstd, dx, dadd, st);
    hipLaunchKernelGGL(skp_gn_bwd_stats_kernel, dim3(a.nsplit, N * G), dim3(256), 0, st, a, dy, mean, rstd, workspace);
    rc = skp_launch_status();
    if (rc) return rc;
    long blocks = (a.L / 4 + 256 * 8 - 1) / (256 * 8);
    if (blocks < 1) blocks = 1;
    if (blocks > 64) blocks = 64;
    hipLaunchKernelGGL(skp_gn_bwd_apply_kernel, dim3((unsigned)blocks, N * G), dim3(256), 0, st, a, dy, mean, rstd,
                       (const float*)workspace, dx, dadd);
    return skp_launch_status();
}

__global__ __launch_bounds__(256) void skp_add_bias_residual_kernel(const float* __restrict__ a, const float* __restrict__ b,
                                                                    const float* __restrict__ bias, float* __restrict__ out,
                                                                    int C, int hw4, long total4) {
    for (long i = (long)blockIdx.x * 256 + threadIdx.x; i < total4; i += (long)gridDim.x * 256) {
        const int c = (int)((i / hw4) % C);
        const f32x4 va = *(const f32x4*)(a + i * 4), vb = *(const f32x4*)(b + i * 4);
        *(f32x4*)(out + i * 4) = va + vb + bias[c];
    }
}

extern "C" int skp_add_bias_residual_f32(const float* a, const float* b, const float* bias, float* out, int N, int C,
                                         int HW, void* stream) {
    if (!a || !b || !bias || !out || N <= 0 || C <= 0 || HW <= 0) return SKP_E_BADARG;
    if (HW % 4) return SKP_E_RANGE;
    const long total4 = (long)N * C * HW / 4;
    long blocks = (total4 + 256 * 4 - 1) / (256 * 4);
    if (blocks > 8192) blocks = 8192;
    hipLaunchKernelGGL(skp_add_bias_residual_kernel, dim3((unsigned)blocks), dim3(256), 0, (hipStream_t)stream, a, b, bias,
                       out, C, HW / 4, total4);
    return skp_launch_status();
}

__device__ __forceinline__ float skp_gelu(float g) { return 0.5f * g * (1.f + erff(g * 0.70710678118654752f)); }
__device__ __forceinline__ float skp_gelu_grad(float g) {
    return 0.5f * (1.f + erff(g * 0.70710678118654752f)) + g * 0.3989422804014327f * __expf(-0.5f * g * g);
}

__global__ __launch_bounds__(256) void skp_geglu_fwd_kernel(const float* __restrict__ p, float* __restrict__ y, int inner4,
                                                            long total4) {
    for (long i = (long)blockIdx.x * 256 + threadIdx.x; i < total4; i += (long)gridDim.x * 256) {
        const long row = i / inner4;
        const int c4 = (int)(i - row * inner4);
        const f32x4* pr = (const f32x4*)p + row * (2 * inner4);
        const f32x4 h = pr[c4], g = pr[inner4 + c4];
        f32x4 o;
#pragma unroll
        for (int j = 0; j < 4; ++j) o[j] = h[j] * skp_gelu(g[j]);
        ((f32x4*)y)[i] = o;
    }
}

__global__ __launch_bounds__(256) void skp_geglu_bwd_kernel(const float* __restrict__ p, const float* __restrict__ dy,
                                                            float* __restrict__ dp, int inner4, long total4) {
    for (long i = (long)blockIdx.x * 256 + threadIdx.x; i < total4; i += (long)gridDim.x * 256) {
        const long row = i / inner4;
        const int c4 = (int)(i - row * inner4);
        const f32x4* pr = (const f32x4*)p + row * (2 * inner4);
        f32x4* dr = (f32x4*)dp + row * (2 * inner4);
        const f32x4 h = pr[c4], g = pr[inner4 + c4], d = ((const f32x4*)dy)[i];
        f32x4 dh, dg;
#pragma unroll
        for (int j = 0; j < 4; ++j) {
            dh[j] = d[j] * skp_gelu(g[j]);
            dg[j] = d[j] * h[j] * skp_gelu_grad(g[j]);
        }
// ... 94 lines not shown
```

stablekeypoints_amd/csrc/skp_select_loss.hip:

```cpp
#include "skp_common.h"
#include <string.h>

__device__ __forceinline__ bool skp_better(float v, int i, float bv, int bi) {
    return (v > bv) || (v == bv && i < bi);
}

struct StatsArgs { int T, R, S; float sigma, eps; };

__global__ __launch_bounds__(256) void skp_token_stats_kernel(const float* __restrict__ M, StatsArgs a,
                                                              int32_t* __restrict__ argmax_out,
                                                              float* __restrict__ kl_out, float* __restrict__ ent_out) {
    __shared__ float red_v[4];
    __shared__ int red_i[4];
    __shared__ float red[4];
    __shared__ float s_cy[SKP_MAX_SUBJECTS], s_cx[SKP_MAX_SUBJECTS];
    const int t = blockIdx.x, tid = threadIdx.x, R = a.R, RR = R * R;
    const float* m = M + (size_t)t * RR;
    const float rad = 0.05f * (float)R;
    const float rad2 = rad * rad;
    float maxval0 = 0.f;
    for (int j = 0; j < a.S; ++j) {
        float bv = -INFINITY; int bi = 0x7fffffff;
        for (int p = tid; p < RR; p += 256) {
            const int row = p / R, col = p - row * R;
// ... 218 lines not shown
    b.wy1 = __fsub_rn(fy, y0f); b.wy0 = __fsub_rn(1.0f, b.wy1);
    return b;
}

__global__ __launch_bounds__(256) void skp_losses_kernel(const float* __restrict__ M, const float* __restrict__ Mt,
                                                         const int64_t* __restrict__ sel,
                                                         const int32_t* __restrict__ argmax, LossArgs a_in,
                                                         float* __restrict__ partial, float* __restrict__ g_sharp,
                                                         float* __restrict__ g_eq_a) {
    __shared__ float red[4];
    const LossArgs a = skp_loss_args(a_in);
    const int k = blockIdx.y, chunk = blockIdx.x, tid = threadIdx.x;
    const int R = a.R, RR = R * R;
    const int tok = (int)sel[k];
    const float* m = M + (size_t)tok * RR;
    const float* mt = Mt + (size_t)tok * RR;
    float pcy[SKP_MAX_SUBJECTS], pcx[SKP_MAX_SUBJECTS];
    for (int j = 0; j < a.S; ++j) {
        const int flat = argmax[j * a.T + tok];
        pcy[j] = __fmul_rn(__fdiv_rn((float)(flat / R) + 0.5f, (float)R), (float)R);
        pcx[j] = __fmul_rn(__fdiv_rn((float)(flat % R) + 0.5f, (float)R), (float)R);
    }
    const float two_sig2 = 2.0f * a.sigma * a.sigma;
    const float inv_S = 1.0f / (float)a.S;
    const float gscale = 2.0f / ((float)a.K * (float)RR);
    float ss = 0.f, se = 0.f;
    for (int u = 0; u < 4; ++u) {
        const int p = chunk * 1024 + u * 256 + tid;
        if (p >= RR) break;
        const int row = p / R, col = p - row * R;
        const float v = m[p];
        float g = 0.f;
        for (int j = 0; j < a.S; ++j) {
            const float dx = (float)col + 0.5f - pcx[j], dy = (float)row + 0.5f - pcy[j];
            g += expf(-(dx * dx + dy * dy) / two_sig2);
        }
        const float ds = v - g * inv_S;
        ss += ds * ds;
        g_sharp[(size_t)k * RR + p] = gscale * ds;
        const SkpBilin bl = skp_bilin(a, col, row);
        const int x0 = bl.x0, y0 = bl.y0, x1 = x0 + 1, y1 = y0 + 1;
        const bool vx0 = x0 >= 0 && x0 < R, vx1 = x1 >= 0 && x1 < R, vy0 = y0 >= 0 && y0 < R, vy1 = y1 >= 0 && y1 < R;
        float sval = 0.f;
        if (vy0 && vx0) sval += mt[y0 * R + x0] * __fmul_rn(bl.wy0, bl.wx0);
        if (vy0 && vx1) sval += mt[y0 * R + x1] * __fmul_rn(bl.wy0, bl.wx1);
        if (vy1 && vx0) sval += mt[y1 * R + x0] * __fmul_rn(bl.wy1, bl.wx0);
        if (vy1 && vx1) sval += mt[y1 * R + x1] * __fmul_rn(bl.wy1, bl.wx1);
        const float de = v - sval;
        se += de * de;
        g_eq_a[(size_t)k * RR + p] = gscale * de;
    }
    ss = skp_block_sum_256(ss, red);
    se = skp_block_sum_256(se, red);
    if (tid == 0) {
        partial[(size_t)(0 * a.K + k) * a.nchunk + chunk] = ss;
        partial[(size_t)(1 * a.K + k) * a.nchunk + chunk] = se;
    }
}

__global__ __launch_bounds__(256) void skp_equiv_grad_kernel(LossArgs a_in, const float* __restrict__ g_eq_a,
                                                            float* __restrict__ g_eq_b) {
    const LossArgs a = skp_loss_args(a_in);
    const int k = blockIdx.y, R = a.R, RR = R * R;
    const int s = blockIdx.x * 256 + threadIdx.x;
    if (s >= RR) return;
    const int sy = s / R, sx = s - sy * R;
    const float a00 = a.th[0], a01 = a.th[1], a10 = a.th[3], a11 = a.th[4];
    const float ox = 0.5f * (float)R * (a.th[2] + 1.0f - a00 - a01) - 0.5f;
    const float oy = 0.5f * (float)R * (a.th[5] + 1.0f - a10 - a11) - 0.5f;
    const float det = a00 * a11 - a01 * a10;
    int c0 = 0, c1 = R - 1, r0 = 0, r1 = R - 1;
    if (fabsf(det) > 1e-12f) {
        const float i00 = a11 / det, i01 = -a01 / det, i10 = -a10 / det, i11 = a00 / det;
        float cmin = INFINITY, cmax = -INFINITY, rmin = INFINITY, rmax = -INFINITY;
#pragma unroll
        for (int q = 0; q < 4; ++q) {
            const float fx = (float)sx + ((q & 1) ? 1.0f : -1.0f) - ox, fy = (float)sy + ((q & 2) ? 1.0f : -1.0f) - oy;
            const float c = i00 * fx + i01 * fy - 0.5f, r = i10 * fx + i11 * fy - 0.5f;
            cmin = fminf(cmin, c); cmax = fmaxf(cmax, c); rmin = fminf(rmin, r); rmax = fmaxf(rmax, r);
        }
        if (cmin == cmin && cmax == cmax && rmin == rmin && rmax == rmax) {
            c0 = (int)fmaxf(floorf(cmin) - 1.0f, 0.0f); c1 = (int)fminf(ceilf(cmax) + 1.0f, (float)(R - 1));
            r0 = (int)fmaxf(floorf(rmin) - 1.0f, 0.0f); r1 = (int)fminf(ceilf(rmax) + 1.0f, (float)(R - 1));
        }
    }
    const float* ga = g_eq_a + (size_t)k * RR;
    float acc = 0.f;
    for (int row = r0; row <= r1; ++row)
        for (int col = c0; col <= c1; ++col) {
            const SkpBilin bl = skp_bilin(a, col, row);
            const float wx = (bl.x0 == sx) ? bl.wx0 : ((bl.x0 + 1 == sx) ? bl.wx1 : 0.f);
            const float wy = (bl.y0 == sy) ? bl.wy0 : ((bl.y0 + 1 == sy) ? bl.wy1 : 0.f);
            const bool hit = (bl.x0 == sx || bl.x0 + 1 == sx) && (bl.y0 == sy || bl.y0 + 1 == sy);
            if (hit) acc -= ga[row * R + col] * __fmul_rn(wy, wx);
        }
    g_eq_b[(size_t)k * RR + s] = acc;
}

static int losses_run(const float* M, const float* Mt, const int64_t* sel, int K, int T, int R, const int32_t* argmax, int num_subjects,
                      float sigma, const float* theta_inv_host, const float* theta_inv_dev, float* partial, float* g_sharp,
                      float* g_eq_a, float* g_eq_b, void* stream) {
    if (!M || !Mt || !sel || !argmax || (!theta_inv_host && !theta_inv_dev) || !partial || !g_sharp || !g_eq_a || !g_eq_b) return SKP_E_BADARG;
    if (K <= 0 || T <= 0 || R <= 0) return SKP_E_BADARG;
    if (num_subjects < 1 || num_subjects > SKP_MAX_SUBJECTS || K > 65535) return SKP_E_RANGE;
    LossArgs a{};
    a.K = K; a.T = T; a.R = R; a.S = num_subjects; a.sigma = sigma;
    a.nchunk = (R * R + 1023) / 1024;
    a.th_dev = theta_inv_dev;
    if (theta_inv_host)
        for (int i = 0; i < 6; ++i) a.th[i] = theta_inv_host[i];
    hipLaunchKernelGGL(skp_losses_kernel, dim3(a.nchunk, K), dim3(256), 0, (hipStream_t)stream, M, Mt, sel, argmax, a,
                       partial, g_sharp, g_eq_a);
    int rc = skp_launch_status();
    if (rc) return rc;
    hipLaunchKernelGGL(skp_equiv_grad_kernel, dim3((R * R + 255) / 256, K), dim3(256), 0, (hipStream_t)stream, a, g_eq_a,
                       g_eq_b);
    return skp_launch_status();
}

extern "C" int skp_losses_fwd_f32(const float* M, const float* Mt, const int64_t* sel, int K, int T, int R,
                                  const int32_t* argmax, int num_subjects, float sigma, const float* theta_inv,
                                  float* partial, float* g_sharp, float* g_eq_a, float* g_eq_b, void* stream) {
    return losses_run(M, Mt, sel, K, T, R, argmax, num_subjects, sigma, theta_inv, nullptr, partial, g_sharp, g_eq_a, g_eq_b, stream);
}

extern "C" int skp_losses_fwd_dev_f32(const float* M, const float* Mt, const int64_t* sel, int K, int T, int R,
                                      const int32_t* argmax, int num_subjects, float sigma, const float* theta_inv_dev,
                                      float* partial, float* g_sharp, float* g_eq_a, float* g_eq_b, void* stream) {
    if (!theta_inv_dev) return SKP_E_BADARG;
    return losses_run(M, Mt, sel, K, T, R, argmax, num_subjects, sigma, nullptr, theta_inv_dev, partial, g_sharp, g_eq_a, g_eq_b, stream);
}

__global__ __launch_bounds__(256) void skp_rows_axpy_kernel(float* __restrict__ dst, const int64_t* __restrict__ sel,
                                                            int64_t n, const float* __restrict__ x,
                                                            const float* __restrict__ a, const float* __restrict__ y,
                                                            const float* __restrict__ b) {
    const int k = blockIdx.y;
    const int64_t i = (int64_t)blockIdx.x * 256 + threadIdx.x;
    if (i >= n) return;
    float v = a[0] * x[(size_t)k * n + i];
    if (y) v += b[0] * y[(size_t)k * n + i];
    dst[(size_t)sel[k] * n + i] += v;
}

extern "C" int skp_rows_axpy_f32(float* dst, const int64_t* sel, int K, int64_t n, const float* x, const float* a,
                                 const float* y, const float* b, void* stream) {
    if (!dst || !sel || !x || !a || K <= 0 || n <= 0 || (y && !b)) return SKP_E_BADARG;
    if (K > 65535) return SKP_E_RANGE;
    hipLaunchKernelGGL(skp_rows_axpy_kernel, dim3((unsigned)((n + 255) / 256), K), dim3(256), 0, (hipStream_t)stream,
                       dst, sel, n, x, a, y, b);
    return skp_launch_status();
}

extern "C" int skp_abi_version(void) { return 39; }

static int g_tune[SKP_TUNE_COUNT] = {0};
static const char* const g_tune_names[SKP_TUNE_COUNT] = {"wino_split", "wino_raw_max_tiles", "map_bands", "fa2_two_kernel_bwd", "gn_fold_max_cout", "cross_attn_ts"};
int skp_tune(int key) { return (key >= 0 && key < SKP_TUNE_COUNT) ? g_tune[key] : 0; }
extern "C" int skp_tune_set(const char* key, int value) {
    if (!key || value < 0) return SKP_E_BADARG;
    for (int i = 0; i < SKP_TUNE_COUNT; ++i)
        if (!strcmp(key, g_tune_names[i])) { g_tune[i] = value; return 0; }
    return SKP_E_RANGE;
}
extern "C" int skp_tune_get(const char* key) {
    if (!key) return SKP_E_BADARG;
    for (int i = 0; i < SKP_TUNE_COUNT; ++i)
        if (!strcmp(key, g_tune_names[i])) return g_tune[i];
    return SKP_E_RANGE;
}
```

stablekeypoints_amd/csrc/skp_wino4_common.h:

```cpp
#pragma once
#include <type_traits>
#include <utility>
#include "skp_common.h"

namespace {

struct Wino4Args {
    const float* x;
    const float* U;
    const float* bias;
    const float* res;
    float* y;
    int B, Cin, Cout, H, W;
    int tilesX, tilesPerImg, nTiles;
    unsigned x_bytes, u_bytes, y_bytes;
    int steps;
    int total_steps;
    int ntb, ncg, tb_per_xcd;
    int splits;
    int gx, vtotal;
    size_t y_split_stride;
    float* stats;
    int sblk;
    const float* gncoef;
    int vpad;
};

__device__ __forceinline__ void w4_park_stats(f32x2* sbuf, int slot, int lane, const f32x4 (&o)[4], bool ok) {
    const float K = o[0][0];
    float s1 = 0.f, s2 = 0.f;
#pragma unroll
    for (int oy = 0; oy < 4; ++oy)
#pragma unroll
        for (int ox = 0; ox < 4; ++ox) { const float d = o[oy][ox] - K; s1 += d; s2 += d * d; }
    const float dm = s1 * (1.0f / 16.0f);
    sbuf[slot * 64 + lane] = ok ? f32x2{K + dm, s2 - s1 * dm} : f32x2{0.f, 0.f};
}
__device__ __forceinline__ void w4_store_stats(const Wino4Args& a, const f32x2* sbuf, int slot, int kq, int tile_first, int co) {
    float msum = 0.f, m2 = 0.f;
#pragma unroll
    for (int i = 0; i < 16; ++i) { const f32x2 t = sbuf[slot * 64 + kq * 16 + i]; msum += t[0]; m2 += t[1]; }
    const float mean = msum * (1.0f / 16.0f);
    float dev = 0.f;
#pragma unroll
    for (int i = 0; i < 16; ++i) { const float d = sbuf[slot * 64 + kq * 16 + i][0] - mean; dev += d * d; }
    if (co < a.Cout && tile_first < a.nTiles) {
        const int b = tile_first / a.tilesPerImg, blk = (tile_first - b * a.tilesPerImg) >> 4;
        *(f32x2*)(a.stats + (((size_t)b * a.Cout + co) * a.sblk + blk) * 2) = f32x2{mean, m2 + 16.0f * dev};
    }
}

__device__ __forceinline__ bool w4_work(const Wino4Args& a, int vid, int& tblock, int& cg, int& z) {
    if (a.tb_per_xcd > 0) {
        z = vid / a.gx;
        const int x = vid - z * a.gx;
        const int xcd = x & 7, seq = x >> 3;
        const int tb_local = seq / a.ncg;
        cg = seq - tb_local * a.ncg;
        tblock = xcd * a.tb_per_xcd + tb_local;
        return tblock < a.ntb;
    }
    const int xcd = vid & 7, q = vid >> 3;
    const int ul = q / a.ntb;
    tblock = q - ul * a.ntb;
    const int u = ul * 8 + xcd;
    z = u / a.ncg;
    cg = u - z * a.ncg;
    return u < a.ncg * a.splits;
}

constexpr int W4_STAGE_F4 = 36 * 4 * 32;
constexpr int W4_RING = 12;

template <class T>
__device__ __forceinline__ void w4_in1d(const T (&d)[6], T (&t)[6]) {
    const T a = d[4] - 4.f * d[2], b = d[3] - 4.f * d[1];
    const T c = d[4] - d[2], e = 2.f * (d[3] - d[1]);
    t[0] = 4.f * d[0] - 5.f * d[2] + d[4];
    t[1] = a + b;
    t[2] = a - b;
    t[3] = c + e;
    t[4] = c - e;
    t[5] = 4.f * d[1] - 5.f * d[3] + d[5];
}
__device__ __forceinline__ void w4_out1d(const float (&m)[6], float (&y)[4]) {
    const float s12 = m[1] + m[2], d12 = m[1] - m[2], s34 = m[3] + m[4], d34 = m[3] - m[4];
    y[0] = m[0] + s12 + s34;
    y[1] = d12 + 2.f * d34;
    y[2] = s12 + 4.f * s34;
    y[3] = d12 + 8.f * d34 + m[5];
}

__global__ void skp_wino4_reduce_kernel(const float* __restrict__ part, const float* __restrict__ bias,
                                        const float* __restrict__ res, float* __restrict__ y, size_t n4, size_t stride,
                                        int splits, int HW4, int Cout) {
    const size_t i = (size_t)blockIdx.x * blockDim.x + threadIdx.x;
    if (i >= n4) return;
    f32x4 acc = ((const f32x4*)part)[i];
    for (int z = 1; z < splits; ++z) acc += ((const f32x4*)(part + z * stride))[i];
    if (bias) {
        const float bv = bias[(i / HW4) % Cout];
        acc += f32x4{bv, bv, bv, bv};
    }
    if (res) acc += ((const f32x4*)res)[i];
    ((f32x4*)y)[i] = acc;
}

struct Wino4Grid { int ntb, ncg, tb_per_xcd; unsigned gx; int rounds; };

#define W4_AGPR_CLOBBERS "a0","a1","a2","a3","a4","a5","a6","a7","a8","a9","a10","a11","a12","a13","a14","a15","a16","a17","a18","a19","a20","a21","a22","a23","a24","a25","a26","a27","a28","a29","a30","a31","a32","a33","a34","a35","a36","a37","a38","a39","a40","a41","a42","a43","a44","a45","a46","a47","a48","a49","a50","a51","a52","a53","a54","a55","a56","a57","a58","a59","a60","a61","a62","a63","a64","a65","a66","a67","a68","a69","a70","a71","a72","a73","a74","a75","a76","a77","a78","a79","a80","a81","a82","a83","a84","a85","a86","a87","a88","a89","a90","a91","a92","a93","a94","a95","a96","a97","a98","a99","a100","a101","a102","a103","a104","a105","a106","a107","a108","a109","a110","a111","a112","a113","a114","a115","a116","a117","a118","a119","a120","a121","a122","a123","a124","a125","a126","a127","a128","a129","a130","a131","a132","a133","a134","a135","a136","a137","a138","a139","a140","a141","a142","a143","a144","a145","a146","a147","a148","a149","a150","a151","a152","a153","a154","a155","a156","a157","a158","a159","a160","a161","a162","a163","a164","a165","a166","a167","a168","a169","a170","a171","a172","a173","a174","a175","a176","a177","a178","a179","a180","a181","a182","a183","a184","a185","a186","a187","a188","a189","a190","a191","a192","a193","a194","a195","a196","a197","a198","a199","a200","a201","a202","a203","a204","a205","a206","a207","a208","a209","a210","a211","a212","a213","a214","a215","a216","a217","a218","a219","a220","a221","a222","a223","a224","a225","a226","a227","a228","a229","a230","a231","a232","a233","a234","a235","a236","a237","a238","a239","a240","a241","a242","a243","a244","a245","a246","a247","a248","a249","a250","a251","a252","a253","a254","a255"
template <int R>
__device__ __forceinline__ float w4_acc_read() {
    float v;
    asm volatile("v_accvgpr_read_b32 %0, a[%1]" : "=v"(v) : "n"(R));
    return v;
}
template <class F, int... I>
__device__ __forceinline__ void w4_unroll(F&& f, std::integer_sequence<int, I...>) { (f(std::integral_constant<int, I>{}), ...); }



}
```

stablekeypoints_amd/ldm/fused.py:

```python
from __future__ import annotations

import torch
import torch.nn.functional as F

from .. import ops
from .attention import AttentionBlock, BasicTransformerBlock, Transformer2DModel
from .unet import Downsample2D, ResnetBlock2D, UNet2DConditionModel


def _resnet_forward(m: ResnetBlock2D):
    orig = m.forward

    def forward(x, temb=None):
        if not ops.group_norm_supported(x, m.norm1.num_groups):
            return orig(x, temb)
        if ops.conv3x3_gn_fold_ok(x, m.norm1, m.conv1.weight):
            h = ops.conv3x3_gn_silu(x, m.norm1, m.conv1.weight, want_stats=True)
        else:
            h, x = ops.group_norm_silu_fork(x, m.norm1)
            h = ops.conv3x3_auto(h, m.conv1.weight, want_stats=True)
        off = _norm2_offset(m, x.shape[0], temb)
        bias = m.conv2.bias
        res = x
        if m.conv_shortcut is not None:
            res, bias = ops.conv1x1_nobias(x, m.conv_shortcut.weight), _summed_bias(m)
        if ops.conv3x3_gn_fold_ok(h, m.norm2, m.conv2.weight, off, bias, res):
            return ops.conv3x3_gn_silu(h, m.norm2, m.conv2.weight, off=off, bias=bias, residual=res, want_stats=True)
        h = ops.group_norm_silu(h, m.norm2, off=off)
        return ops.conv3x3_auto(h, m.conv2.weight, bias, residual=res, want_stats=True)
    return forward


def _norm2_offset(m: ResnetBlock2D, rows: int, temb):
    def build():
        off = m.conv1.bias[None, :].expand(rows, -1)
        if m.time_emb_proj is not None and temb is not None:
            off = off + m.time_emb_proj(F.silu(temb))
        return off.contiguous()
    proj = m.time_emb_proj.parameters() if m.time_emb_proj is not None else ()
    return ops.cached(m, ("norm2_offset", rows), (m.conv1.bias, *proj, temb), build)


def _time_path(m: UNet2DConditionModel):
    orig = m.time_path

    def time_path(sample, timestep, added_cond_kwargs=None):
        host = not torch.is_tensor(timestep) or (timestep.device.type == "cpu" and timestep.numel() <= 64)
        tag = ops.frozen_tag([*m.time_embedding.parameters(), *(m.add_embedding.parameters() if m.add_embedding is not None else ())])
        if not host or tag is None or added_cond_kwargs is not None:
            return orig(sample, timestep, added_cond_kwargs)
        vals = tuple(float(v) for v in (timestep.reshape(-1).tolist() if torch.is_tensor(timestep) else [timestep]))
        key = (vals, int(sample.shape[0]), tuple(sample.shape[-2:]), sample.device, sample.dtype, tag)
        memo = m.__dict__.setdefault("_skp_temb", {})
        hit = memo.get(key)
        if hit is None:
            if len(memo) >= 8:
                memo.clear()
            with torch.no_grad():
                hit = orig(sample, timestep, added_cond_kwargs)
            memo[key] = hit
        return ops.handed_out(hit)
    return time_path


def _summed_bias(m: ResnetBlock2D):
    b2, bs = m.conv2.bias, m.conv_shortcut.bias
    if bs is None:
        return b2
    return ops.cached(m, "bias_sum", (b2, bs), lambda: b2 + bs)


def _transformer_forward(m: Transformer2DModel):
    orig = m.forward

    def forward(x, context=None):
        if not ops.group_norm_supported(x, m.norm.num_groups):
            return orig(x, context)
        if not ops.layout_supported(x):
            return orig(x, context)
        h, x = ops.group_norm_silu_fork(x, m.norm, silu=False)
        t = ops.nchw_to_tokens(h)
        t = F.linear(t, m.proj_in.weight.flatten(1), m.proj_in.bias)
        for blk in m.transformer_blocks:
            t = blk(t, context=context)
        t = F.linear(t, m.proj_out.weight.flatten(1), m.proj_out.bias)
        return ops.tokens_to_nchw_add(t, x)
    return forward


def _block_forward(m: BasicTransformerBlock):
    orig = m.forward

    def forward(h, context=None):
        if not (ops.add_layer_norm_supported(h, m.norm1) and ops.add_layer_norm_supported(h, m.norm2)
                and ops.add_layer_norm_supported(h, m.norm3)):
            return orig(h, context=context)
        h, n = ops.add_layer_norm(None, h, m.norm1)
        h, n = ops.add_layer_norm(m.attn1(n), h, m.norm2)
        h, n = ops.add_layer_norm(m.attn2(n, context=context), h, m.norm3)
        return m.ff(n) + h
    return forward


def _vae_attention_forward(m: AttentionBlock):
    orig = m.forward

    def forward(x):
        if not (ops.group_norm_supported(x, m.group_norm.num_groups) and ops.layout_supported(x)):
            return orig(x)
        b, c, hh, ww = x.shape
        t = ops.nchw_to_tokens(ops.group_norm_silu(x, m.group_norm, silu=False))
        q, k, v = m.query(t), m.key(t), m.value(t)
        nh = m.num_heads
        d = c // nh

        def split(u):
            return u.reshape(b, -1, nh, d).permute(0, 2, 1, 3).reshape(b * nh, -1, d)
        q, k, v = split(q), split(k), split(v)
        attn = torch.baddbmm(torch.empty(q.shape[0], q.shape[1], k.shape[1], dtype=q.dtype, device=q.device),
                             q, k.transpose(1, 2), beta=0, alpha=1.0 / (d ** 0.5)).softmax(dim=-1)
        o = torch.bmm(attn, v).reshape(b, nh, -1, d).permute(0, 2, 1, 3).reshape(b, -1, c)
        return ops.tokens_to_nchw_add(m.proj_attn(o), x)
    return forward


def _conv_forward(m: torch.nn.Conv2d):
    def forward(x):
        return ops.conv3x3_auto(x, m.weight, m.bias, want_stats=m.weight.shape[1] <= 4)
    return forward


def _downsample_forward(m):
    orig = m.forward

    def forward(x):
        frozen = not (m.conv.weight.requires_grad or (m.conv.bias is not None and m.conv.bias.requires_grad))
        if frozen and m.conv.stride == (2, 2) and ops.conv3x3_s2_supported(x, m.conv.weight):
            return ops.conv3x3_s2(x, m.conv.weight, m.conv.bias, pad=0 if m.padding == 0 else 1, want_stats=True)
        return orig(x)
    return forward


def _vae_encode(m):
    orig = m.encode
    from .vae import DiagonalGaussianDistribution

    def compose():
        enc, q = m.encoder, m.quant_conv
        with torch.no_grad():
            wq = q.weight.flatten(1).double()
            w = (wq @ enc.conv_out.weight.double().flatten(1)).reshape(q.weight.shape[0], *enc.conv_out.weight.shape[1:])
            b = wq @ enc.conv_out.bias.double() + q.bias.double()
            co = w.shape[0]
            wp = torch.zeros(32, *w.shape[1:], device=w.device, dtype=torch.float32)
            bp = torch.zeros(32, device=w.device, dtype=torch.float32)
            wp[:co], bp[:co] = w.float(), b.float()
        return wp, bp

    def tail_params():
        return (m.encoder.conv_out.weight, m.encoder.conv_out.bias, m.quant_conv.weight, m.quant_conv.bias)

    def encode(x):
        enc, q = m.encoder, m.quant_conv
        ok = (x.is_cuda and x.dtype == torch.float32 and not torch.is_grad_enabled() and q.kernel_size == (1, 1)
              and q.weight.shape[0] <= 32 and enc.conv_out.kernel_size == (3, 3) and enc.conv_out.padding == (1, 1)
              and q.bias is not None and enc.conv_out.bias is not None and not any(p.requires_grad for p in tail_params()))
        if not ok:
            return orig(x)
        h = enc.conv_in(x)
        for blk in enc.down_blocks:
            h = blk(h)
        h = enc.mid_block(h)
        if not (ops.group_norm_supported(h, enc.conv_norm_out.num_groups) and ops.conv3x3_wanted(h.shape, (32, h.shape[1], 3, 3))):
            return {"latent_dist": DiagonalGaussianDistribution(q(enc.conv_out(F.silu(enc.conv_norm_out(h)))))}
        wp, bp = ops.cached(m, "vae_tail", tail_params(), compose)
        h = ops.group_norm_silu(h, enc.conv_norm_out)
        y = ops.conv3x3_auto(h, wp, bp)
        return {"latent_dist": DiagonalGaussianDistribution(y[:, :q.weight.shape[0]])}
    return encode


def fuse_norms(module: torch.nn.Module) -> int:
    n = 0
# ... 27 lines not shown
```

stablekeypoints_amd/ops.py:

```python
from __future__ import annotations

import contextlib
import weakref
from typing import List, Sequence, Tuple

import torch

from . import _native as N


def _stream() -> int:
    return torch.cuda.current_stream().cuda_stream


def _dev(t: torch.Tensor, name: str) -> torch.Tensor:
    if not t.is_cuda:
        raise RuntimeError(f"{name}: the StableKeypoints hot path runs on the HIP kernels only "
                           f"(got a {t.device} tensor; there is no CPU fallback)")
    if t.dtype != torch.float32:
        raise RuntimeError(f"{name}: expected float32, got {t.dtype}")
    return t if t.is_contiguous() else t.contiguous()


def _ptr(t):
# ... 830 lines not shown


def _wino4r_filters(weight, backward):
    return _filters(weight, "f4r", backward)


def _conv3x3_raw(x, U, bias, cout, variant=0, split=True, residual=None, out=None):
    B, ci, H, W = x.shape
    y = out if out is not None else torch.empty(B, cout, H, W, device=x.device, dtype=torch.float32)
    ws = _workspace("skp_conv3x3_workspace", B, ci, cout, H, W, int(variant), device=x.device) if split else None
    N.check(N.lib().skp_conv3x3_f32(x.data_ptr(), U.data_ptr(), _ptr(bias), _ptr(residual), y.data_ptr(), _ptr(ws),
                                    B, ci, cout, H, W, int(variant), _stream()), "skp_conv3x3_f32")
    return y


def _conv3x3_f4_raw(x, U, bias, cout, split=True, residual=None, out=None, stats=None):
    B, ci, H, W = x.shape
    y = out if out is not None else torch.empty(B, cout, H, W, device=x.device, dtype=torch.float32)
    if stats is not None:
        N.check(N.lib().skp_conv3x3_f4_stats_f32(x.data_ptr(), U.data_ptr(), _ptr(bias), _ptr(residual), y.data_ptr(),
                                                 stats.data_ptr(), B, ci, cout, H, W, _stream()), "skp_conv3x3_f4_stats_f32")
        return y
    ws = _workspace("skp_conv3x3_f4_workspace", B, ci, cout, H, W, device=x.device) if split else None
    N.check(N.lib().skp_conv3x3_f4_f32(x.data_ptr(), U.data_ptr(), _ptr(bias), _ptr(residual), y.data_ptr(), _ptr(ws),
                                       B, ci, cout, H, W, _stream()), "skp_conv3x3_f4_f32")
    return y


def _conv3x3_f4r_raw(x, R, bias, cout, residual=None, out=None):
    B, ci, H, W = x.shape
    y = out if out is not None else torch.empty(B, cout, H, W, device=x.device, dtype=torch.float32)
    ws = _workspace("skp_conv3x3_f4r_workspace", B, ci, cout, H, W, device=x.device)
    N.check(N.lib().skp_conv3x3_f4r_f32(x.data_ptr(), R.data_ptr(), _ptr(bias), _ptr(residual), y.data_ptr(), _ptr(ws),
                                        B, ci, cout, H, W, _stream()), "skp_conv3x3_f4r_f32")
    return y


def conv3x3_f4r_ok(x_shape, cout) -> bool:
    b, ci, h, w = (int(v) for v in x_shape)
    return CONV3X3_MODE == "f4" and bool(N.lib().skp_conv3x3_f4r_ok(b, ci, int(cout), h, w))


CONV3X3_MODE = "f4"


def conv3x3_f4_ok(x_shape, w_shape):
    b, _, h, w = (int(v) for v in x_shape)
    if not (CONV3X3_MODE == "f4" and h % 4 == 0 and w % 4 == 0 and int(w_shape[0]) % 16 == 0 and int(w_shape[1]) % 16 == 0
            and 36 * int(w_shape[0]) * int(w_shape[1]) * 4 < 2 ** 31):
        return False
    return b * (h // 4) * (w // 4) >= 32 or conv3x3_f4r_ok(x_shape, int(w_shape[0]))


def conv3x3_wanted(x_shape, w_shape):
    if CONV3X3_MODE == "lib" or not conv3x3_supported(x_shape, w_shape):
        return False
    b, _, h, w = (int(v) for v in x_shape)
    return conv3x3_f4_ok(x_shape, w_shape) or b * ((h + 1) // 2) * ((w + 1) // 2) >= 128


def conv3x3_stats_blocks(x_shape, w_shape) -> int:
    if not (GN_FUSED_STATS and conv3x3_f4_ok(x_shape, w_shape)):
        return 0
    b, ci, h, w = (int(v) for v in x_shape)
    co = int(w_shape[0])
    if max(ci, co) * h * w * 4 * b >= 2 ** 31:
        return 0
    return int(N.lib().skp_conv3x3_f4_stats_blocks(b, ci, co, h, w))


def _rows_per_launch(ci, co, H, W) -> int:
    return max(1, (2 ** 31 - 1) // (max(ci, co) * H * W * 4))


def _conv3x3_run(x, weight, backward, bias, residual, cout, stats=None):
    w_shape = (weight.shape[1], weight.shape[0], 3, 3) if backward else weight.shape
    f4 = conv3x3_f4_ok(x.shape, w_shape)
    B, ci, H, W = x.shape
    if f4 and stats is None and conv3x3_f4r_ok(x.shape, cout):
        return _conv3x3_f4r_raw(x, _filters(weight, "f4r", backward), bias, cout, residual=residual)
    U = _filters(weight, "f4" if f4 else "f2", backward)
    run = _conv3x3_f4_raw if f4 else _conv3x3_raw
    chunk = _rows_per_launch(ci, cout, H, W)
    if stats is not None:
        return _conv3x3_f4_raw(x, U, bias, cout, residual=residual, stats=stats)
    if B <= chunk:
        return run(x, U, bias, cout, residual=residual)
    y = torch.empty(B, cout, H, W, device=x.device, dtype=torch.float32)
    for b0 in range(0, B, chunk):
        b1 = min(B, b0 + chunk)
        run(x[b0:b1], U, bias, cout, residual=None if residual is None else residual[b0:b1], out=y[b0:b1])
    return y


class Conv3x3Fn(torch.autograd.Function):

    @staticmethod
    def forward(ctx, x, weight, bias, residual=None, stats=None):
        x = _dev(x, "x")
        ctx.weight = weight
        if residual is not None:
            residual = _dev(residual, "residual")
        return _conv3x3_run(x, weight, False, bias, residual, weight.shape[0], stats=stats)

    @staticmethod
    def backward(ctx, dy):
        dx = None
        if ctx.needs_input_grad[0]:
            w = ctx.weight
            co, ci = w.shape[:2]
            if conv3x3_wanted(dy.shape, (ci, co, 3, 3)):
                dx = _conv3x3_run(_dev(dy, "dy"), w, True, None, None, ci)
            else:
                dx = torch.nn.grad.conv2d_input((dy.shape[0], ci, dy.shape[2], dy.shape[3]), w, dy, padding=1)
        return dx, None, None, (dy if ctx.needs_input_grad[3] else None), None


def conv3x3(x, weight, bias=None, residual=None):
    if not conv3x3_supported(x.shape, weight.shape):
        raise ValueError(f"conv3x3: unsupported shape x {tuple(x.shape)} w {tuple(weight.shape)}")
    if weight.requires_grad or (bias is not None and bias.requires_grad):
        raise ValueError("conv3x3: the Winograd kernels serve FROZEN weights only (no weight/bias gradient)")
    return Conv3x3Fn.apply(x, weight, bias, residual)


GN_ONEPASS = True


def _stats_useful(cout: int, h: int, w: int, groups: int = 32, rows: int = 1) -> bool:
    return not (GN_ONEPASS and cout % groups == 0 and N.lib().skp_group_norm_onepass_ok(int(rows), int(cout), int(groups), int(h * w)))


def conv3x3_auto(x, weight, bias=None, residual=None, want_stats=False):
    frozen = not (weight.requires_grad or (bias is not None and bias.requires_grad))
    if frozen and x.is_cuda and x.dtype == torch.float32 and conv3x3_wanted(x.shape, weight.shape):
        nblk = conv3x3_stats_blocks(x.shape, weight.shape) if (want_stats and _stats_useful(weight.shape[0], x.shape[2], x.shape[3])) else 0
        if nblk:
            stats = torch.empty(x.shape[0], weight.shape[0], nblk, 2, device=x.device, dtype=torch.float32)
            y = Conv3x3Fn.apply(x, weight, bias, residual, stats)
            y._skp_blocks = (stats, nblk, 256)
            return y
        return Conv3x3Fn.apply(x, weight, bias, residual)
    if (frozen and residual is None and x.is_cuda and x.dtype == torch.float32 and CONV3X3_MODE != "lib"
            and weight.shape[1] <= 4 and x.shape[3] % 2 == 0 and not (torch.is_grad_enabled() and x.requires_grad)):
        return conv3x3_small(x, weight, bias, want_stats=want_stats)
    if residual is None:
        return torch.nn.functional.conv2d(x, weight, bias, padding=1)
    y = torch.nn.functional.conv2d(x, weight, None, padding=1)
    if bias is not None and y.is_cuda and y.dtype == torch.float32 and (y.shape[2] * y.shape[3]) % 4 == 0:
        return add_bias_residual(residual, y, bias)
    return (y + bias[None, :, None, None] if bias is not None else y) + residual


GN_FOLD = True


def conv3x3_gn_fold_ok(x, norm: torch.nn.GroupNorm, weight, *others) -> bool:
    if not (GN_FOLD and x.is_cuda and x.dtype == torch.float32):
        return False
    if torch.is_grad_enabled() and any(t_ is not None and t_.requires_grad
                                       for t_ in (x, weight, norm.weight, norm.bias, *others)):
        return False
    if weight.requires_grad or not conv3x3_f4_ok(x.shape, weight.shape) or not group_norm_supported(x, norm.num_groups):
        return False
    B, ci, H, W = x.shape
    co = int(weight.shape[0])
    rows = min(B, _rows_per_launch(ci, co, H, W))
    return bool(N.lib().skp_conv3x3_f4_gn_ok(rows, ci, co, H, W)) and (B % rows == 0 or bool(
        N.lib().skp_conv3x3_f4_gn_ok(B % rows, ci, co, H, W)))


@torch.no_grad()
def conv3x3_gn_silu(x, norm: torch.nn.GroupNorm, weight, off=None, bias=None, residual=None, want_stats=False):
    x = _dev(x, "x")
    B, C, H, W = x.shape
    G, cout = norm.num_groups, int(weight.shape[0])
    off_c = _dev(off.reshape(B, C), "off") if off is not None else None
    bias = _dev(bias, "bias") if bias is not None else None
    residual = _dev(residual, "residual") if residual is not None else None
    if residual is not None and tuple(residual.shape) != (B, cout, H, W):
        raise RuntimeError("conv3x3_gn_silu: residual must have the output's shape")
    mean = torch.empty(B, G, device=x.device, dtype=torch.float32)
    rstd = torch.empty_like(mean)
    coef = torch.empty(B, C, 2, device=x.device, dtype=torch.float32)
    blocks = _blocks(x)
    lib, st = N.lib(), _stream()
    if blocks is not None:
        bs, nblk, pix = blocks
        N.check(lib.skp_group_norm_coef_f32(None, off_c.data_ptr() if off_c is not None else None, norm.weight.data_ptr(),
                                            norm.bias.data_ptr(), mean.data_ptr(), rstd.data_ptr(), coef.data_ptr(),
                                            bs.data_ptr(), int(nblk), int(pix), None, B, C, G, H * W, float(norm.eps), st),
                "skp_group_norm_coef_f32")
    else:
        ws = torch.empty(B * G * 64 * 3, device=x.device, dtype=torch.float32)
        N.check(lib.skp_group_norm_coef_f32(x.data_ptr(), off_c.data_ptr() if off_c is not None else None,
                                            norm.weight.data_ptr(), norm.bias.data_ptr(), mean.data_ptr(), rstd.data_ptr(),
                                            coef.data_ptr(), None, 0, 0, ws.data_ptr(), B, C, G, H * W, float(norm.eps), st),
                "skp_group_norm_coef_f32")
    U = _filters(weight, "f4")
    y = torch.empty(B, cout, H, W, device=x.device, dtype=torch.float32)
    nblk = conv3x3_stats_blocks(x.shape, weight.shape) if (want_stats and _stats_useful(cout, H, W)) else 0
    stats = torch.empty(B, cout, nblk, 2, device=x.device, dtype=torch.float32) if nblk else None
    chunk = _rows_per_launch(C, cout, H, W)
    for b0 in range(0, B, chunk):
        b1 = min(B, b0 + chunk)
        N.check(lib.skp_conv3x3_f4_gn_f32(x[b0:b1].data_ptr(), U.data_ptr(), bias.data_ptr() if bias is not None else None,
                                          residual[b0:b1].data_ptr() if residual is not None else None, y[b0:b1].data_ptr(),
                                          stats[b0:b1].data_ptr() if stats is not None else None, coef[b0:b1].data_ptr(),
                                          b1 - b0, C, cout, H, W, st), "skp_conv3x3_f4_gn_f32")
    if stats is not None:
        y._skp_blocks = (stats, nblk, 256)
    return y


def conv3x3_small(x, weight, bias=None, want_stats=False):
    x, w = _dev(x.detach(), "x"), _dev(weight.detach(), "weight")
    B, ci, H, W = x.shape
    y = torch.empty(B, w.shape[0], H, W, device=x.device, dtype=torch.float32)
    bb = _dev(bias.detach(), "bias") if bias is not None else None
    nblk = int(N.lib().skp_conv3x3_small_stats_blocks(B, ci, w.shape[0], H, W)) if (want_stats and GN_FUSED_STATS) else 0
    if nblk:
        stats = torch.empty(B, w.shape[0], nblk, 2, device=x.device, dtype=torch.float32)
        N.check(N.lib().skp_conv3x3_small_stats_f32(x.data_ptr(), w.data_ptr(), bb.data_ptr() if bb is not None else None, y.data_ptr(),
                                                    stats.data_ptr(), B, ci, w.shape[0], H, W, _stream()), "skp_conv3x3_small_stats_f32")
        y._skp_blocks = (stats, nblk, 512)
        return y
    N.check(N.lib().skp_conv3x3_small_f32(x.data_ptr(), w.data_ptr(), bb.data_ptr() if bb is not None else None, y.data_ptr(),
                                          B, ci, w.shape[0], H, W, _stream()), "skp_conv3x3_small_f32")
    return y


def mfma_issue_rate(waves_per_simd: int = 1, iters: int = 20000, device=None) -> float:
    import ctypes
    dev = torch.device("cuda", torch.cuda.current_device()) if device is None else torch.device(device)
    scratch = torch.empty(256 * 4 * 256, device=dev, dtype=torch.float32)
    out = ctypes.c_float(0.0)
    with torch.cuda.device(dev):
        N.check(N.lab().skp_probe_mfma_f32(int(waves_per_simd), int(iters), scratch.data_ptr(), ctypes.addressof(out), _stream()),
                "skp_probe_mfma_f32")
    return float(out.value)


def _qkv_stack(wq, wk, wv):
    return weight_stack([wq, wk, wv])


def weight_stack(ws):
    return cached(ws[0], ("stack", *map(id, ws)), ws, lambda: torch.stack([w.detach() for w in ws]).contiguous())


QKV_STACKED = True


def _qkv_forward(x, wq, wk, wv):
    F = torch.nn.functional
    if not (QKV_STACKED and x.is_cuda and wq.shape == wk.shape == wv.shape):
        return F.linear(x, wq), F.linear(x, wk), F.linear(x, wv)
    c_in, c_out = wq.shape[1], wq.shape[0]
    x2 = x.reshape(-1, c_in)
    m = x2.shape[0]
    out = torch.bmm(x2.unsqueeze(0).expand(3, m, c_in), _qkv_stack(wq, wk, wv).transpose(1, 2))
    shp = (*x.shape[:-1], c_out)
    return out[0].view(shp), out[1].view(shp), out[2].view(shp)


class QKVProjFn(torch.autograd.Function):

    @staticmethod
    def forward(ctx, x, wq, wk, wv):
        ctx.save_for_backward(wq, wk, wv)
        return _qkv_forward(x, wq, wk, wv)

    @staticmethod
    def backward(ctx, dq, dk, dv):
        wq, wk, wv = ctx.saved_tensors
        shp = dq.shape
        dx = torch.mm(dq.reshape(-1, shp[-1]), wq)
        dx.addmm_(dk.reshape(-1, shp[-1]), wk)
        dx.addmm_(dv.reshape(-1, shp[-1]), wv)
        return dx.reshape(*shp[:-1], wq.shape[1]), None, None, None


QKV_ACCUM = True


def qkv_proj(x, wq, wk, wv):
    frozen = not (wq.requires_grad or wk.requires_grad or wv.requires_grad)
    if QKV_ACCUM and x.is_cuda and x.requires_grad and torch.is_grad_enabled() and frozen:
        return QKVProjFn.apply(x, wq, wk, wv)
    if frozen and not (x.requires_grad and torch.is_grad_enabled()):
        return _qkv_forward(x, wq, wk, wv)
    F = torch.nn.functional
    return F.linear(x, wq), F.linear(x, wk), F.linear(x, wv)


class SelfAttnQKVFn(torch.autograd.Function):

    @staticmethod
    def forward(ctx, x, wq, wk, wv, heads, scale):
        q, k, v = _qkv_forward(x, wq, wk, wv)
        B, Nq, C = q.shape
        out = torch.empty_like(q)
        lse = torch.empty(B, heads, Nq, device=q.device, dtype=torch.float32)
        _flash_fwd(q, k, v, out, lse, heads, scale)
        ctx.save_for_backward(q, k, v, out, lse, wq, wk, wv)
        ctx.meta = (int(heads), float(scale), tuple(x.shape))
# ... 175 lines not shown
```

Before: 53.27.

## Fuse split-K conv partial reduction and Winograd input transform into GroupNorm

Adds a fused ResNet inner path (conv1 -> GroupNorm+SiLU -> conv2) for grad-enabled forward and its backward. The conv writes raw split-K partials, and the GroupNorm kernel sums them itself, removing the separate reduce launch. The GroupNorm kernel also emits the Winograd F(4,3) input tiles for the next conv, so that conv skips its own input-transform kernel. The cost is extra work and workspace inside the GroupNorm kernels, plus added complexity in a custom autograd function.

```diff
diff --git a/include/skp.h b/include/skp.h
--- a/include/skp.h
+++ b/include/skp.h
@@ -70,6 +70,16 @@
 int64_t skp_conv3x3_f4r_workspace(int B, int Cin, int Cout, int H, int W);
 int skp_conv3x3_f4r_f32(const void* x, const void* R, const void* bias, const void* residual, void* y, void* workspace,
                         int B, int Cin, int Cout, int H, int W, void* stream);
+
+int64_t skp_conv3x3_f4_part_workspace(int B, int Cin, int Cout, int H, int W);
+int skp_conv3x3_f4_part_f32(const void* x, const void* U, void* part, int B, int Cin, int Cout, int H, int W, void* stream);
+int64_t skp_conv3x3_f4r_part_workspace(int B, int Cin, int Cout, int H, int W);
+int skp_conv3x3_f4r_part_f32(const void* x, const void* R, void* part, void* workspace, int B, int Cin, int Cout, int H, int W,
+                             void* stream);
+int64_t skp_conv3x3_f4r_tiles_workspace(int B, int Cin, int H, int W);
+int64_t skp_conv3x3_f4r_pre_workspace(int B, int Cin, int Cout, int H, int W);
+int skp_conv3x3_f4r_pre_f32(const void* V, const void* R, const void* bias, const void* residual, void* y, void* workspace,
+                            int B, int Cin, int Cout, int H, int W, void* stream);
 
 int skp_cross_attn_fwd_f32(const float* q, const float* k, const float* v, float* out, float* lse,
                            int B, int Bk, int H, int N, int T, int d, float scale, void* stream);
@@ -116,6 +126,13 @@
                            float* mean, float* rstd, float* workspace, int N, int C, int G, int HW, float eps,
                            int silu, void* stream);
 int skp_group_norm_onepass_ok(int N, int C, int G, int HW);
+int skp_group_norm_parts_ok(int N, int C, int G, int H, int W, int tiles);
+int skp_group_norm_fwd_parts_f32(const float* part, int S, float* xsum, const float* off, const float* gamma, const float* beta,
+                                 float* y, float* tiles, float* mean, float* rstd, int N, int C, int G, int H, int W, float eps,
+                                 int silu, void* stream);
+int skp_group_norm_bwd_parts_f32(const float* x, const float* off, const float* gamma, const float* beta, const float* dpart, int S,
+                                 const float* mean, const float* rstd, float* dx, float* tiles, int N, int C, int G, int H, int W,
+                                 float eps, int silu, void* stream);
 int skp_group_norm_bwd_f32(const float* x, const float* off, const float* gamma, const float* beta,
                            const float* dy, const float* mean, const float* rstd, float* dx, float* workspace,
                            int N, int C, int G, int HW, float eps, int silu, void* stream);
diff --git a/stablekeypoints_amd/_native.py b/stablekeypoints_amd/_native.py
--- a/stablekeypoints_amd/_native.py
+++ b/stablekeypoints_amd/_native.py
@@ -7,7 +7,7 @@
 
 _HERE = os.path.dirname(os.path.abspath(__file__))
 LIB_PATH = os.environ.get("SKP_LIB_PATH") or os.path.join(_HERE, "csrc", "libskp_hip.so")
-ABI_VERSION = 39
+ABI_VERSION = 40
 
 _vp, _i, _f, _i64 = C.c_void_p, C.c_int, C.c_float, C.c_int64
 
@@ -71,6 +71,16 @@
     "skp_conv3x3_f4r_filter_f32": [_vp, _vp, _i, _i, _i, _vp],
     "skp_conv3x3_f4r_workspace": [_i, _i, _i, _i, _i],
     "skp_conv3x3_f4r_f32": [_vp, _vp, _vp, _vp, _vp, _vp, _i, _i, _i, _i, _i, _vp],
+    "skp_conv3x3_f4_part_workspace": [_i, _i, _i, _i, _i],
+    "skp_conv3x3_f4_part_f32": [_vp, _vp, _vp, _i, _i, _i, _i, _i, _vp],
+    "skp_conv3x3_f4r_part_workspace": [_i, _i, _i, _i, _i],
+    "skp_conv3x3_f4r_part_f32": [_vp, _vp, _vp, _vp, _i, _i, _i, _i, _i, _vp],
+    "skp_conv3x3_f4r_tiles_workspace": [_i, _i, _i, _i],
+    "skp_conv3x3_f4r_pre_workspace": [_i, _i, _i, _i, _i],
+    "skp_conv3x3_f4r_pre_f32": [_vp, _vp, _vp, _vp, _vp, _vp, _i, _i, _i, _i, _i, _vp],
+    "skp_group_norm_parts_ok": [_i, _i, _i, _i, _i, _i],
+    "skp_group_norm_fwd_parts_f32": [_vp, _i, _vp, _vp, _vp, _vp, _vp, _vp, _vp, _vp, _i, _i, _i, _i, _i, _f, _i, _vp],
+    "skp_group_norm_bwd_parts_f32": [_vp, _vp, _vp, _vp, _vp, _i, _vp, _vp, _vp, _vp, _i, _i, _i, _i, _i, _f, _i, _vp],
     "skp_conv3x3_s2_filter_f32": [_vp, _vp, _i, _i, _vp],
     "skp_conv3x3_s2_f32": [_vp, _vp, _vp, _vp, _i, _i, _i, _i, _i, _i, _vp],
     "skp_conv3x3_s2_workspace": [_i, _i, _i, _i, _i],
diff --git a/stablekeypoints_amd/csrc/skp_conv_wino4.hip b/stablekeypoints_amd/csrc/skp_conv_wino4.hip
--- a/stablekeypoints_amd/csrc/skp_conv_wino4.hip
+++ b/stablekeypoints_amd/csrc/skp_conv_wino4.hip
@@ -289,41 +289,7 @@
     const int m = idx & 3, rest = idx >> 2;
     const int tg = rest % vpad, q4 = rest / vpad;
     if (q4 >= (Cin >> 2)) return;
-    const bool tv = tg < nTiles;
-    const int tgc = tv ? tg : 0;
-    const int b = tgc / tilesPerImg, rem = tgc - b * tilesPerImg;
-    const int ty = rem / tilesX, tx = rem - ty * tilesX;
-    const float dsc[6] = {0.25f, -1.f / 6, -1.f / 6, 1.f / 24, 1.f / 24, 1.f};
-    const float* xc = x + ((size_t)b * Cin + q4 * 4 + m) * H * W;
-    float d[6][6];
-#pragma unroll
-    for (int i = 0; i < 6; ++i) {
-        const int r = 4 * ty - 1 + i;
-        const bool rv = tv && r >= 0 && r < H;
-        const float* row = xc + r * W + 4 * tx;
-        const f32x4 mid = rv ? *(const f32x4*)row : f32x4{0.f, 0.f, 0.f, 0.f};
-        d[i][0] = (rv && tx > 0) ? row[-1] : 0.f;
-        d[i][1] = mid[0]; d[i][2] = mid[1]; d[i][3] = mid[2]; d[i][4] = mid[3];
-        d[i][5] = (rv && tx + 1 < tilesX) ? row[4] : 0.f;
-    }
-#pragma unroll
-    for (int j = 0; j < 6; ++j) {
-        float v[6], t[6];
-#pragma unroll
-        for (int i = 0; i < 6; ++i) v[i] = d[i][j];
-        w4_in1d(v, t);
-#pragma unroll
-        for (int i = 0; i < 6; ++i) d[i][j] = t[i];
-    }
-    const int c16 = q4 >> 2, kq = q4 & 3;
-    float* dst = Vg + (((size_t)c16 * 36 * 4 + kq) * vpad + tg) * 4 + m;
-#pragma unroll
-    for (int i = 0; i < 6; ++i) {
-        float t[6];
-        w4_in1d(d[i], t);
-#pragma unroll
-        for (int j = 0; j < 6; ++j) dst[(size_t)(i * 6 + j) * 16 * vpad] = t[j] * (dsc[i] * dsc[j]);
-    }
+    w4r_input_tile(x, Vg, Cin, H, W, tilesX, tilesPerImg, nTiles, vpad, q4, m, tg);
 }
 
 #ifdef W4R_STAMPS
@@ -927,7 +893,7 @@
 }
 
 static int wino4_run(const void* x, const void* U, const void* bias, const void* residual, void* y, void* workspace, float* stats,
-                     int B, int Cin, int Cout, int H, int W, void* stream, const float* gncoef = nullptr);
+                     int B, int Cin, int Cout, int H, int W, void* stream, const float* gncoef = nullptr, void* part = nullptr);
 
 extern "C" int skp_conv3x3_f4_gn_ok(int B, int Cin, int Cout, int H, int W) {
     if (wino4_plan(B, Cin, Cout, H, W) != 1) return 0;
@@ -949,6 +915,15 @@
     return wino4_run(x, U, bias, residual, y, workspace, nullptr, B, Cin, Cout, H, W, stream);
 }
 
+extern "C" int64_t skp_conv3x3_f4_part_workspace(int B, int Cin, int Cout, int H, int W) {
+    return (int64_t)wino4_plan(B, Cin, Cout, H, W) * B * Cout * H * W * (int64_t)sizeof(float);
+}
+
+extern "C" int skp_conv3x3_f4_part_f32(const void* x, const void* U, void* part, int B, int Cin, int Cout, int H, int W, void* stream) {
+    if (!part) return SKP_E_BADARG;
+    return wino4_run(x, U, nullptr, nullptr, nullptr, nullptr, nullptr, B, Cin, Cout, H, W, stream, nullptr, part);
+}
+
 extern "C" int skp_conv3x3_f4_stats_f32(const void* x, const void* U, const void* bias, const void* residual, void* y,
                                         float* stats, int B, int Cin, int Cout, int H, int W, void* stream) {
     if (!stats || skp_conv3x3_f4_stats_blocks(B, Cin, Cout, H, W) == 0) return SKP_E_RANGE;
@@ -956,11 +931,11 @@
 }
 
 static int wino4_run(const void* x, const void* U, const void* bias, const void* residual, void* y, void* workspace, float* stats,
-                     int B, int Cin, int Cout, int H, int W, void* stream, const float* gncoef) {
-    if (!x || !U || !y) return SKP_E_BADARG;
+                     int B, int Cin, int Cout, int H, int W, void* stream, const float* gncoef, void* part) {
+    if (!x || !U || !(y || part)) return SKP_E_BADARG;
     int S = wino4_plan(B, Cin, Cout, H, W);
     if (S == 0) return (B <= 0 || Cin <= 0 || Cout <= 0 || H <= 0 || W <= 0) ? SKP_E_BADARG : SKP_E_RANGE;
-    if (!workspace) S = 1;
+    if (!workspace && !part) S = 1;
     const unsigned long long xb = (unsigned long long)B * Cin * H * W * 4, ub = (unsigned long long)36 * Cin * Cout * 4,
                              yb = (unsigned long long)B * Cout * H * W * 4;
     if (xb >= 0x80000000ull || ub >= 0x80000000ull || yb >= 0x80000000ull) return SKP_E_RANGE;
@@ -976,10 +951,10 @@
     a.splits = S;
     const size_t out_elems = (size_t)B * Cout * H * W;
     a.y_split_stride = out_elems;
-    a.y = S > 1 ? (float*)workspace : (float*)y;
-    a.bias = S > 1 ? nullptr : (const float*)bias;
-    a.res = S > 1 ? nullptr : (const float*)residual;
-    a.stats = S > 1 ? nullptr : stats;
+    a.y = part ? (float*)part : S > 1 ? (float*)workspace : (float*)y;
+    a.bias = (part || S > 1) ? nullptr : (const float*)bias;
+    a.res = (part || S > 1) ? nullptr : (const float*)residual;
+    a.stats = (part || S > 1) ? nullptr : stats;
     a.sblk = a.tilesPerImg / 16;
     a.gncoef = gncoef;
     hipStream_t st = (hipStream_t)stream;
@@ -1025,7 +1000,7 @@
         else hipLaunchKernelGGL(skp_wino4_conv_kernel<false>, grid, dim3(256), lds, st, a);
     }
     int rc = skp_launch_status();
-    if (rc || S == 1) return rc;
+    if (rc || S == 1 || part) return rc;
     const size_t n4 = out_elems / 4;
     hipLaunchKernelGGL(skp_wino4_reduce_kernel, dim3((unsigned)((n4 + 255) / 256)), dim3(256), 0, st, (const float*)workspace,
                        (const float*)bias, (const float*)residual, (float*)y, n4, out_elems, S, (H * W) / 4, Cout);
@@ -1052,9 +1027,26 @@
     return 36 * (int64_t)Cin * vpad * 4 + (S > 1 ? (int64_t)S * B * Cout * H * W * 4 : 0);
 }
 
-extern "C" int skp_conv3x3_f4r_f32(const void* x, const void* R, const void* bias, const void* residual, void* y, void* workspace,
-                                   int B, int Cin, int Cout, int H, int W, void* stream) {
-    if (!x || !R || !y || !workspace) return SKP_E_BADARG;
+extern "C" int64_t skp_conv3x3_f4r_tiles_workspace(int B, int Cin, int H, int W) {
+    if (B <= 0 || Cin <= 0 || H <= 0 || W <= 0 || (Cin % 16) || (H % 4) || (W % 4)) return 0;
+    const int64_t tiles = (int64_t)B * (H / 4) * (W / 4), vpad = (tiles + 31) / 32 * 32;
+    return 36 * (int64_t)Cin * vpad * 4;
+}
+
+extern "C" int64_t skp_conv3x3_f4r_pre_workspace(int B, int Cin, int Cout, int H, int W) {
+    if (!wino4r_layout_ok(B, Cin, Cout, H, W)) return 0;
+    const int S = wino4r_plan(B, Cin, Cout, H, W);
+    return S > 1 ? (int64_t)S * B * Cout * H * W * 4 : 0;
+}
+
+extern "C" int64_t skp_conv3x3_f4r_part_workspace(int B, int Cin, int Cout, int H, int W) {
+    if (!wino4r_layout_ok(B, Cin, Cout, H, W)) return 0;
+    return (int64_t)wino4r_plan(B, Cin, Cout, H, W) * B * Cout * H * W * 4;
+}
+
+static int wino4r_run(const void* x, const void* Vin, const void* R, const void* bias, const void* residual, void* y, void* part,
+                      void* ws, int B, int Cin, int Cout, int H, int W, void* stream) {
+    if (!(x || Vin) || !R || !(y || part)) return SKP_E_BADARG;
     if (!wino4r_layout_ok(B, Cin, Cout, H, W)) return (B <= 0 || Cin <= 0 || Cout <= 0 || H <= 0 || W <= 0) ? SKP_E_BADARG : SKP_E_RANGE;
     const int S = wino4r_plan(B, Cin, Cout, H, W);
     Wino4Args a;
@@ -1064,8 +1056,9 @@
     a.nTiles = B * a.tilesPerImg;
     a.vpad = (a.nTiles + 31) / 32 * 32;
     const size_t v_elems = (size_t)36 * Cin * a.vpad;
-    float* Vg = (float*)workspace;
-    float* part = Vg + v_elems;
+    float* Vg = Vin ? (float*)Vin : (float*)ws;
+    float* sp = Vin ? (float*)ws : (float*)ws + v_elems;
+    if (!Vg || (!part && S > 1 && !ws)) return SKP_E_BADARG;
     a.x = Vg; a.U = (const float*)R;
     a.x_bytes = (unsigned)(v_elems * 4); a.u_bytes = (unsigned)((size_t)9 * Cin * Cout * 4);
     const size_t out_elems = (size_t)B * Cout * H * W;
@@ -1074,9 +1067,9 @@
     a.steps = (a.total_steps + S - 1) / S;
     a.splits = S;
     a.y_split_stride = out_elems;
-    a.y = S > 1 ? part : (float*)y;
-    a.bias = S > 1 ? nullptr : (const float*)bias;
-    a.res = S > 1 ? nullptr : (const float*)residual;
+    a.y = part ? (float*)part : S > 1 ? sp : (float*)y;
+    a.bias = (part || S > 1) ? nullptr : (const float*)bias;
+    a.res = (part || S > 1) ? nullptr : (const float*)residual;
     a.stats = nullptr; a.sblk = 0; a.gncoef = nullptr;
     hipStream_t st = (hipStream_t)stream;
     const size_t lds = (size_t)2 * W4_STAGE_F4 * sizeof(f32x4);
@@ -1096,9 +1089,11 @@
     a.ntb = g.ntb; a.ncg = g.ncg; a.tb_per_xcd = g.tb_per_xcd;
     a.gx = (int)g.gx;
     a.vtotal = g.tb_per_xcd ? (int)g.gx * S : (int)g.gx;
-    const int nin = a.vpad * Cin;
-    hipLaunchKernelGGL(skp_wino4r_input_kernel, dim3((unsigned)((nin + 255) / 256)), dim3(256), 0, st, (const float*)x, Vg, B, Cin, H, W,
-                       a.tilesX, a.tilesPerImg, a.nTiles, a.vpad);
+    if (!Vin) {
+        const int nin = a.vpad * Cin;
+        hipLaunchKernelGGL(skp_wino4r_input_kernel, dim3((unsigned)((nin + 255) / 256)), dim3(256), 0, st, (const float*)x, Vg, B, Cin, H,
+                           W, a.tilesX, a.tilesPerImg, a.nTiles, a.vpad);
+    }
     const dim3 grid = g.tb_per_xcd ? dim3(g.gx, 1, S) : dim3(g.gx, 1, 1);
     if (a.nTiles <= 16) {
         if (S > 1) hipLaunchKernelGGL((skp_wino4r_conv_kernel<true, 1>), grid, dim3(256), lds, st, a);
@@ -1106,11 +1101,29 @@
     } else if (S > 1) hipLaunchKernelGGL(skp_wino4r_conv_kernel<true>, grid, dim3(256), lds, st, a);
     else hipLaunchKernelGGL(skp_wino4r_conv_kernel<false>, grid, dim3(256), lds, st, a);
     int rc = skp_launch_status();
-    if (rc || S == 1) return rc;
+    if (rc || S == 1 || part) return rc;
     const size_t n4 = out_elems / 4;
-    hipLaunchKernelGGL(skp_wino4_reduce_kernel, dim3((unsigned)((n4 + 255) / 256)), dim3(256), 0, st, (const float*)part,
+    hipLaunchKernelGGL(skp_wino4_reduce_kernel, dim3((unsigned)((n4 + 255) / 256)), dim3(256), 0, st, (const float*)sp,
                        (const float*)bias, (const float*)residual, (float*)y, n4, out_elems, S, (H * W) / 4, Cout);
     return skp_launch_status();
+}
+
+extern "C" int skp_conv3x3_f4r_f32(const void* x, const void* R, const void* bias, const void* residual, void* y, void* workspace,
+                                   int B, int Cin, int Cout, int H, int W, void* stream) {
+    if (!x || !workspace) return SKP_E_BADARG;
+    return wino4r_run(x, nullptr, R, bias, residual, y, nullptr, workspace, B, Cin, Cout, H, W, stream);
+}
+
+extern "C" int skp_conv3x3_f4r_pre_f32(const void* V, const void* R, const void* bias, const void* residual, void* y, void* workspace,
+                                       int B, int Cin, int Cout, int H, int W, void* stream) {
+    if (!V) return SKP_E_BADARG;
+    return wino4r_run(nullptr, V, R, bias, residual, y, nullptr, workspace, B, Cin, Cout, H, W, stream);
+}
+
+extern "C" int skp_conv3x3_f4r_part_f32(const void* x, const void* R, void* part, void* workspace, int B, int Cin, int Cout, int H,
+                                        int W, void* stream) {
+    if (!x || !part || !workspace) return SKP_E_BADARG;
+    return wino4r_run(x, nullptr, R, nullptr, nullptr, nullptr, part, workspace, B, Cin, Cout, H, W, stream);
 }
 
 #ifdef W4R_STAMPS
diff --git a/stablekeypoints_amd/csrc/skp_group_norm.hip b/stablekeypoints_amd/csrc/skp_group_norm.hip
--- a/stablekeypoints_amd/csrc/skp_group_norm.hip
+++ b/stablekeypoints_amd/csrc/skp_group_norm.hip
@@ -1,4 +1,5 @@
 #include "skp_common.h"
+#include "skp_wino4_input.h"
 #include <stdlib.h>
 
 struct GNArgs {
@@ -217,9 +218,34 @@
     return t;
 }
 
-template <int VPT>
+struct GNFuse {
+    const float* part;
+    size_t stride;
+    int S;
+    float* xsum;
+    float* Vg;
+    int H, W, tilesX, tilesPerImg, nTiles, vpad;
+};
+
+__device__ __forceinline__ f32x4 gn_part_sum(const GNFuse& f, size_t o) {
+    f32x4 acc = *(const f32x4*)(f.part + o);
+    for (int z = 1; z < f.S; ++z) acc += *(const f32x4*)(f.part + z * f.stride + o);
+    return acc;
+}
+
+__device__ __forceinline__ void gn_tiles(const GNArgs& a, const GNFuse& f, const float* src, int row) {
+    const int n = row / a.G, g = row - n * a.G, Cg = a.C / a.G;
+    const int t0 = n * f.tilesPerImg, nt = (n == a.N - 1 ? f.vpad : t0 + f.tilesPerImg) - t0;
+    const int items = Cg * nt;
+    for (int k = threadIdx.x; k < items; k += blockDim.x) {
+        const int m = k & 3, rest = k >> 2, tl = rest % nt, ql = rest / nt;
+        w4r_input_tile(src, f.Vg, a.C, f.H, f.W, f.tilesX, f.tilesPerImg, f.nTiles, f.vpad, g * (Cg / 4) + ql, m, t0 + tl);
+    }
+}
+
+template <int VPT, bool FUSE = false>
 __global__ __launch_bounds__(1024) void skp_gn_onepass_fwd_kernel(GNArgs a, float* __restrict__ y, float* __restrict__ mean_out,
-                                                                  float* __restrict__ rstd_out) {
+                                                                  float* __restrict__ rstd_out, GNFuse f) {
     __shared__ float red[16];
     const int row = blockIdx.x, tid = threadIdx.x;
     const int n = row / a.G, g = row - n * a.G, Cg = a.C / a.G;
@@ -233,7 +259,12 @@
         const int i = tid + 1024 * j;
         v[j] = f32x4{0.f, 0.f, 0.f, 0.f};
         if (i < q4) {
-            v[j] = *(const f32x4*)(xr + (size_t)i * 4);
+            if constexpr (FUSE) {
+                v[j] = gn_part_sum(f, (size_t)row * a.L + (size_t)i * 4);
+                if (f.xsum) *(f32x4*)(f.xsum + (size_t)row * a.L + (size_t)i * 4) = v[j];
+            } else {
+                v[j] = *(const f32x4*)(xr + (size_t)i * 4);
+            }
             if (a.off) v[j] += a.off[(size_t)n * a.C + g * Cg + i / hw4];
             s += (v[j][0] + v[j][1]) + (v[j][2] + v[j][3]);
         }
@@ -264,18 +295,23 @@
             *(f32x4*)(yr + (size_t)i * 4) = r;
         }
     }
-}
-
-template <int VPT>
+    if constexpr (FUSE) {
+        if (f.Vg) {
+            __syncthreads();
+            gn_tiles(a, f, y, row);
+        }
+    }
+}
+
+template <int VPT, bool FUSE = false>
 __global__ __launch_bounds__(1024) void skp_gn_onepass_bwd_kernel(GNArgs a, const float* __restrict__ dy, const float* __restrict__ mean_in,
                                                                   const float* __restrict__ rstd_in, float* __restrict__ dx,
-                                                                  const float* __restrict__ dadd) {
+                                                                  const float* __restrict__ dadd, GNFuse f) {
     __shared__ float red[16];
     const int row = blockIdx.x, tid = threadIdx.x;
     const int n = row / a.G, g = row - n * a.G, Cg = a.C / a.G;
     const float mean = mean_in[row], rstd = rstd_in[row];
     const float* xr = a.x + (size_t)row * a.L;
-    const float* dr = dy + (size_t)row * a.L;
     float* dxr = dx + (size_t)row * a.L;
     const int hw4 = a.HW / 4, q4 = (int)(a.L / 4);
     f32x4 xh[VPT], gz[VPT];
@@ -290,7 +326,8 @@
             const float gam = a.gamma[c], bet = a.beta[c];
             const float o = a.off ? a.off[(size_t)n * a.C + c] : 0.f;
             const f32x4 xv = *(const f32x4*)(xr + (size_t)i * 4);
-            const f32x4 dv = *(const f32x4*)(dr + (size_t)i * 4);
+            const size_t o4 = (size_t)row * a.L + (size_t)i * 4;
+            const f32x4 dv = FUSE ? gn_part_sum(f, o4) : *(const f32x4*)(dy + o4);
 #pragma unroll
             for (int e = 0; e < 4; ++e) {
                 const float h = (xv[e] + o - mean) * rstd;
@@ -317,6 +354,12 @@
             *(f32x4*)(dxr + (size_t)i * 4) = r;
         }
     }
+    if constexpr (FUSE) {
+        if (f.Vg) {
+            __syncthreads();
+            gn_tiles(a, f, dx, row);
+        }
+    }
 }
 
 static int gn_onepass_vpt(const GNArgs& a, bool backward) {
@@ -329,14 +372,34 @@
     return 0;
 }
 
-static int gn_onepass_fwd(const GNArgs& a, float* y, float* mean, float* rstd, hipStream_t st) {
+template <bool FUSE>
+static int gn_onepass_fwd_t(const GNArgs& a, float* y, float* mean, float* rstd, const GNFuse& f, hipStream_t st) {
     const dim3 grid(a.N * a.G), block(1024);
     switch (gn_onepass_vpt(a, false)) {
-        case 1: hipLaunchKernelGGL(skp_gn_onepass_fwd_kernel<1>, grid, block, 0, st, a, y, mean, rstd); break;
-        case 2: hipLaunchKernelGGL(skp_gn_onepass_fwd_kernel<2>, grid, block, 0, st, a, y, mean, rstd); break;
-        case 4: hipLaunchKernelGGL(skp_gn_onepass_fwd_kernel<4>, grid, block, 0, st, a, y, mean, rstd); break;
-        case 10: hipLaunchKernelGGL(skp_gn_onepass_fwd_kernel<10>, grid, block, 0, st, a, y, mean, rstd); break;
-        case 16: hipLaunchKernelGGL(skp_gn_onepass_fwd_kernel<16>, grid, block, 0, st, a, y, mean, rstd); break;
+        case 1: hipLaunchKernelGGL((skp_gn_onepass_fwd_kernel<1, FUSE>), grid, block, 0, st, a, y, mean, rstd, f); break;
+        case 2: hipLaunchKernelGGL((skp_gn_onepass_fwd_kernel<2, FUSE>), grid, block, 0, st, a, y, mean, rstd, f); break;
+        case 4: hipLaunchKernelGGL((skp_gn_onepass_fwd_kernel<4, FUSE>), grid, block, 0, st, a, y, mean, rstd, f); break;
+        case 10: hipLaunchKernelGGL((skp_gn_onepass_fwd_kernel<10, FUSE>), grid, block, 0, st, a, y, mean, rstd, f); break;
+        case 16: hipLaunchKernelGGL((skp_gn_onepass_fwd_kernel<16, FUSE>), grid, block, 0, st, a, y, mean, rstd, f); break;
+        default: return -100;
+    }
+    return skp_launch_status();
+}
+
+static int gn_onepass_fwd(const GNArgs& a, float* y, float* mean, float* rstd, hipStream_t st) {
+    return gn_onepass_fwd_t<false>(a, y, mean, rstd, GNFuse{}, st);
+}
+
+template <bool FUSE>
+static int gn_onepass_bwd_t(const GNArgs& a, const float* dy, const float* mean, const float* rstd, float* dx, const float* dadd,
+                            const GNFuse& f, hipStream_t st) {
+    const dim3 grid(a.N * a.G), block(1024);
+    switch (gn_onepass_vpt(a, true)) {
+        case 1: hipLaunchKernelGGL((skp_gn_onepass_bwd_kernel<1, FUSE>), grid, block, 0, st, a, dy, mean, rstd, dx, dadd, f); break;
+        case 2: hipLaunchKernelGGL((skp_gn_onepass_bwd_kernel<2, FUSE>), grid, block, 0, st, a, dy, mean, rstd, dx, dadd, f); break;
+        case 4: hipLaunchKernelGGL((skp_gn_onepass_bwd_kernel<4, FUSE>), grid, block, 0, st, a, dy, mean, rstd, dx, dadd, f); break;
+        case 8: hipLaunchKernelGGL((skp_gn_onepass_bwd_kernel<8, FUSE>), grid, block, 0, st, a, dy, mean, rstd, dx, dadd, f); break;
+        case 10: hipLaunchKernelGGL((skp_gn_onepass_bwd_kernel<10, FUSE>), grid, block, 0, st, a, dy, mean, rstd, dx, dadd, f); break;
         default: return -100;
     }
     return skp_launch_status();
@@ -344,16 +407,7 @@
 
 static int gn_onepass_bwd(const GNArgs& a, const float* dy, const float* mean, const float* rstd, float* dx, const float* dadd,
                           hipStream_t st) {
-    const dim3 grid(a.N * a.G), block(1024);
-    switch (gn_onepass_vpt(a, true)) {
-        case 1: hipLaunchKernelGGL(skp_gn_onepass_bwd_kernel<1>, grid, block, 0, st, a, dy, mean, rstd, dx, dadd); break;
-        case 2: hipLaunchKernelGGL(skp_gn_onepass_bwd_kernel<2>, grid, block, 0, st, a, dy, mean, rstd, dx, dadd); break;
-        case 4: hipLaunchKernelGGL(skp_gn_onepass_bwd_kernel<4>, grid, block, 0, st, a, dy, mean, rstd, dx, dadd); break;
-        case 8: hipLaunchKernelGGL(skp_gn_onepass_bwd_kernel<8>, grid, block, 0, st, a, dy, mean, rstd, dx, dadd); break;
-        case 10: hipLaunchKernelGGL(skp_gn_onepass_bwd_kernel<10>, grid, block, 0, st, a, dy, mean, rstd, dx, dadd); break;
-        default: return -100;
-    }
-    return skp_launch_status();
+    return gn_onepass_bwd_t<false>(a, dy, mean, rstd, dx, dadd, GNFuse{}, st);
 }
 
 static int gn_fill(GNArgs& a, const float* x, const float* off, const float* gamma, const float* beta, int N, int C,
@@ -405,6 +459,49 @@
     return skp_launch_status();
 }
 
+extern "C" int skp_group_norm_parts_ok(int N, int C, int G, int H, int W, int tiles) {
+    if (N <= 0 || C <= 0 || G <= 0 || H <= 0 || W <= 0 || C % G || ((H * W) & 3) || (long)N * G > 65535) return 0;
+    GNArgs a{};
+    a.N = N; a.C = C; a.G = G; a.HW = H * W; a.L = (long)(C / G) * a.HW;
+    if (!gn_onepass_vpt(a, false) || !gn_onepass_vpt(a, true)) return 0;
+    if (tiles && ((C / G) % 4 || C % 16 || H % 4 || W % 4)) return 0;
+    return 1;
+}
+
+static int gn_fuse_fill(GNFuse& f, const float* part, int S, float* xsum, float* Vg, int N, int C, int H, int W) {
+    if (!part || S < 1) return SKP_E_BADARG;
+    f.part = part; f.S = S; f.stride = (size_t)N * C * H * W; f.xsum = xsum; f.Vg = Vg;
+    f.H = H; f.W = W; f.tilesX = W / 4; f.tilesPerImg = (W / 4) * (H / 4); f.nTiles = N * f.tilesPerImg;
+    f.vpad = (f.nTiles + 31) / 32 * 32;
+    return 0;
+}
+
+extern "C" int skp_group_norm_fwd_parts_f32(const float* part, int S, float* xsum, const float* off, const float* gamma,
+                                            const float* beta, float* y, float* tiles, float* mean, float* rstd, int N, int C, int G,
+                                            int H, int W, float eps, int silu, void* stream) {
+    if (!skp_group_norm_parts_ok(N, C, G, H, W, tiles != nullptr)) return SKP_E_RANGE;
+    if (!y || !mean || !rstd || (S > 1 && !xsum)) return SKP_E_BADARG;
+    GNArgs a{};
+    int rc = gn_fill(a, part, off, gamma, beta, N, C, G, H * W, eps, silu);
+    if (rc) return rc;
+    GNFuse f{};
+    if ((rc = gn_fuse_fill(f, part, S, xsum, tiles, N, C, H, W))) return rc;
+    return gn_onepass_fwd_t<true>(a, y, mean, rstd, f, (hipStream_t)stream);
+}
+
+extern "C" int skp_group_norm_bwd_parts_f32(const float* x, const float* off, const float* gamma, const float* beta, const float* dpart,
+                                            int S, const float* mean, const float* rstd, float* dx, float* tiles, int N, int C, int G,
+                                            int H, int W, float eps, int silu, void* stream) {
+    if (!skp_group_norm_parts_ok(N, C, G, H, W, tiles != nullptr)) return SKP_E_RANGE;
+    if (!mean || !rstd || !dx) return SKP_E_BADARG;
+    GNArgs a{};
+    int rc = gn_fill(a, x, off, gamma, beta, N, C, G, H * W, eps, silu);
+    if (rc) return rc;
+    GNFuse f{};
+    if ((rc = gn_fuse_fill(f, dpart, S, nullptr, tiles, N, C, H, W))) return rc;
+    return gn_onepass_bwd_t<true>(a, nullptr, mean, rstd, dx, nullptr, f, (hipStream_t)stream);
+}
+
 extern "C" int skp_group_norm_fwd_blocks_f32(const float* x, const float* off, const float* gamma, const float* beta,
                                              float* y, float* mean, float* rstd, const float* bs, int nblk, int pix, int N, int C,
                                              int G, int HW, float eps, int silu, void* stream) {
diff --git a/stablekeypoints_amd/csrc/skp_select_loss.hip b/stablekeypoints_amd/csrc/skp_select_loss.hip
--- a/stablekeypoints_amd/csrc/skp_select_loss.hip
+++ b/stablekeypoints_amd/csrc/skp_select_loss.hip
@@ -394,7 +394,7 @@
     return skp_launch_status();
 }
 
-extern "C" int skp_abi_version(void) { return 39; }
+extern "C" int skp_abi_version(void) { return 40; }
 
 static int g_tune[SKP_TUNE_COUNT] = {0};
 static const char* const g_tune_names[SKP_TUNE_COUNT] = {"wino_split", "wino_raw_max_tiles", "map_bands", "fa2_two_kernel_bwd", "gn_fold_max_cout", "cross_attn_ts"};
diff --git a/stablekeypoints_amd/csrc/skp_wino4_common.h b/stablekeypoints_amd/csrc/skp_wino4_common.h
--- a/stablekeypoints_amd/csrc/skp_wino4_common.h
+++ b/stablekeypoints_amd/csrc/skp_wino4_common.h
@@ -2,6 +2,7 @@
 #include <type_traits>
 #include <utility>
 #include "skp_common.h"
+#include "skp_wino4_input.h"
 
 namespace {
 
@@ -72,17 +73,6 @@
 constexpr int W4_STAGE_F4 = 36 * 4 * 32;
 constexpr int W4_RING = 12;
 
-template <class T>
-__device__ __forceinline__ void w4_in1d(const T (&d)[6], T (&t)[6]) {
-    const T a = d[4] - 4.f * d[2], b = d[3] - 4.f * d[1];
-    const T c = d[4] - d[2], e = 2.f * (d[3] - d[1]);
-    t[0] = 4.f * d[0] - 5.f * d[2] + d[4];
-    t[1] = a + b;
-    t[2] = a - b;
-    t[3] = c + e;
-    t[4] = c - e;
-    t[5] = 4.f * d[1] - 5.f * d[3] + d[5];
-}
 __device__ __forceinline__ void w4_out1d(const float (&m)[6], float (&y)[4]) {
     const float s12 = m[1] + m[2], d12 = m[1] - m[2], s34 = m[3] + m[4], d34 = m[3] - m[4];
     y[0] = m[0] + s12 + s34;
diff --git a/stablekeypoints_amd/csrc/skp_wino4_input.h b/stablekeypoints_amd/csrc/skp_wino4_input.h
--- /dev/null
+++ b/stablekeypoints_amd/csrc/skp_wino4_input.h
@@ -0,0 +1,57 @@
+#pragma once
+#include "skp_common.h"
+
+namespace {
+
+template <class T>
+__device__ __forceinline__ void w4_in1d(const T (&d)[6], T (&t)[6]) {
+    const T a = d[4] - 4.f * d[2], b = d[3] - 4.f * d[1];
+    const T c = d[4] - d[2], e = 2.f * (d[3] - d[1]);
+    t[0] = 4.f * d[0] - 5.f * d[2] + d[4];
+    t[1] = a + b;
+    t[2] = a - b;
+    t[3] = c + e;
+    t[4] = c - e;
+    t[5] = 4.f * d[1] - 5.f * d[3] + d[5];
+}
+
+__device__ __forceinline__ void w4r_input_tile(const float* __restrict__ x, float* __restrict__ Vg, int Cin, int H, int W, int tilesX,
+                                               int tilesPerImg, int nTiles, int vpad, int q4, int m, int tg) {
+    const bool tv = tg < nTiles;
+    const int tgc = tv ? tg : 0;
+    const int b = tgc / tilesPerImg, rem = tgc - b * tilesPerImg;
+    const int ty = rem / tilesX, tx = rem - ty * tilesX;
+    const float dsc[6] = {0.25f, -1.f / 6, -1.f / 6, 1.f / 24, 1.f / 24, 1.f};
+    const float* xc = x + ((size_t)b * Cin + q4 * 4 + m) * H * W;
+    float d[6][6];
+#pragma unroll
+    for (int i = 0; i < 6; ++i) {
+        const int r = 4 * ty - 1 + i;
+        const bool rv = tv && r >= 0 && r < H;
+        const float* row = xc + r * W + 4 * tx;
+        const f32x4 mid = rv ? *(const f32x4*)row : f32x4{0.f, 0.f, 0.f, 0.f};
+        d[i][0] = (rv && tx > 0) ? row[-1] : 0.f;
+        d[i][1] = mid[0]; d[i][2] = mid[1]; d[i][3] = mid[2]; d[i][4] = mid[3];
+        d[i][5] = (rv && tx + 1 < tilesX) ? row[4] : 0.f;
+    }
+#pragma unroll
+    for (int j = 0; j < 6; ++j) {
+        float v[6], t[6];
+#pragma unroll
+        for (int i = 0; i < 6; ++i) v[i] = d[i][j];
+        w4_in1d(v, t);
+#pragma unroll
+        for (int i = 0; i < 6; ++i) d[i][j] = t[i];
+    }
+    const int c16 = q4 >> 2, kq = q4 & 3;
+    float* dst = Vg + (((size_t)c16 * 36 * 4 + kq) * vpad + tg) * 4 + m;
+#pragma unroll
+    for (int i = 0; i < 6; ++i) {
+        float t[6];
+        w4_in1d(d[i], t);
+#pragma unroll
+        for (int j = 0; j < 6; ++j) dst[(size_t)(i * 6 + j) * 16 * vpad] = t[j] * (dsc[i] * dsc[j]);
+    }
+}
+
+}
diff --git a/stablekeypoints_amd/ldm/fused.py b/stablekeypoints_amd/ldm/fused.py
--- a/stablekeypoints_amd/ldm/fused.py
+++ b/stablekeypoints_amd/ldm/fused.py
@@ -14,21 +14,30 @@
     def forward(x, temb=None):
         if not ops.group_norm_supported(x, m.norm1.num_groups):
             return orig(x, temb)
-        if ops.conv3x3_gn_fold_ok(x, m.norm1, m.conv1.weight):
+        fold1 = ops.conv3x3_gn_fold_ok(x, m.norm1, m.conv1.weight)
+        if fold1:
             h = ops.conv3x3_gn_silu(x, m.norm1, m.conv1.weight, want_stats=True)
         else:
             h, x = ops.group_norm_silu_fork(x, m.norm1)
+        off, bias, res = _conv2_operands(m, x, temb)
+        if not fold1:
+            if ops.resnet_inner_ok(h, m.conv1.weight, m.norm2, m.conv2.weight, off, bias, res):
+                return ops.resnet_inner(h, m.conv1.weight, m.norm2, m.conv2.weight, off=off, bias=bias, residual=res)
             h = ops.conv3x3_auto(h, m.conv1.weight, want_stats=True)
-        off = _norm2_offset(m, x.shape[0], temb)
-        bias = m.conv2.bias
-        res = x
-        if m.conv_shortcut is not None:
-            res, bias = ops.conv1x1_nobias(x, m.conv_shortcut.weight), _summed_bias(m)
         if ops.conv3x3_gn_fold_ok(h, m.norm2, m.conv2.weight, off, bias, res):
             return ops.conv3x3_gn_silu(h, m.norm2, m.conv2.weight, off=off, bias=bias, residual=res, want_stats=True)
         h = ops.group_norm_silu(h, m.norm2, off=off)
         return ops.conv3x3_auto(h, m.conv2.weight, bias, residual=res, want_stats=True)
     return forward
+
+
+def _conv2_operands(m: ResnetBlock2D, x, temb):
+    off = _norm2_offset(m, x.shape[0], temb)
+    bias = m.conv2.bias
+    res = x
+    if m.conv_shortcut is not None:
+        res, bias = ops.conv1x1_nobias(x, m.conv_shortcut.weight), _summed_bias(m)
+    return off, bias, res
 
 
 def _norm2_offset(m: ResnetBlock2D, rows: int, temb):
diff --git a/stablekeypoints_amd/ops.py b/stablekeypoints_amd/ops.py
--- a/stablekeypoints_amd/ops.py
+++ b/stablekeypoints_amd/ops.py
@@ -1006,6 +1006,121 @@
     return (y + bias[None, :, None, None] if bias is not None else y) + residual
 
 
+GN_TAKES_PARTIALS = True
+
+
+def _f4_launch(x_shape, w_shape) -> bool:
+    b, ci, h, w = (int(v) for v in x_shape)
+    return (conv3x3_wanted(x_shape, w_shape) and conv3x3_f4_ok(x_shape, w_shape)
+            and b <= _rows_per_launch(ci, int(w_shape[0]), h, w))
+
+
+def _tiles_ok(B, C, G, H, W, cout) -> bool:
+    return conv3x3_f4r_ok((B, C, H, W), cout) and bool(N.lib().skp_group_norm_parts_ok(B, C, G, H, W, 1))
+
+
+def resnet_inner_ok(h, w1, norm: torch.nn.GroupNorm, w2, off=None, bias=None, residual=None) -> bool:
+    if not (GN_TAKES_PARTIALS and h.is_cuda and h.dtype == torch.float32 and h.dim() == 4 and torch.is_grad_enabled()
+            and h.requires_grad):
+        return False
+    if any(t is not None and t.requires_grad for t in (w1, w2, norm.weight, norm.bias, off, bias)):
+        return False
+    B, C1, H, W = (int(v) for v in h.shape)
+    C, C2, G = int(w1.shape[0]), int(w2.shape[0]), norm.num_groups
+    if int(w1.shape[1]) != C1 or int(w2.shape[1]) != C or (residual is not None and tuple(residual.shape) != (B, C2, H, W)):
+        return False
+    if not (_f4_launch((B, C1, H, W), w1.shape) and _f4_launch((B, C, H, W), w2.shape)
+            and _f4_launch((B, C2, H, W), (C, C2, 3, 3)) and _f4_launch((B, C, H, W), (C1, C, 3, 3))):
+        return False
+    return bool(N.lib().skp_group_norm_parts_ok(B, C, G, H, W, 0)) and not _stats_useful(C2, H, W)
+
+
+def _conv3x3_parts(x, weight, backward, cout):
+    B, ci, H, W = x.shape
+    lib, dev = N.lib(), x.device
+    if conv3x3_f4r_ok(x.shape, cout):
+        R = _filters(weight, "f4r", backward)
+        part = _workspace("skp_conv3x3_f4r_part_workspace", B, ci, cout, H, W, device=dev)
+        ws = _workspace("skp_conv3x3_f4r_tiles_workspace", B, ci, H, W, device=dev)
+        N.check(lib.skp_conv3x3_f4r_part_f32(x.data_ptr(), R.data_ptr(), part.data_ptr(), ws.data_ptr(), B, ci, cout, H, W,
+                                             _stream()), "skp_conv3x3_f4r_part_f32")
+    else:
+        U = _filters(weight, "f4", backward)
+        part = _workspace("skp_conv3x3_f4_part_workspace", B, ci, cout, H, W, device=dev)
+        N.check(lib.skp_conv3x3_f4_part_f32(x.data_ptr(), U.data_ptr(), part.data_ptr(), B, ci, cout, H, W, _stream()),
+                "skp_conv3x3_f4_part_f32")
+    return part, part.numel() // (B * cout * H * W)
+
+
+def _conv3x3_f4r_pre(tiles, weight, backward, bias, residual, shape, cout):
+    B, ci, H, W = shape
+    y = torch.empty(B, cout, H, W, device=tiles.device, dtype=torch.float32)
+    ws = _workspace("skp_conv3x3_f4r_pre_workspace", B, ci, cout, H, W, device=tiles.device)
+    N.check(N.lib().skp_conv3x3_f4r_pre_f32(tiles.data_ptr(), _filters(weight, "f4r", backward).data_ptr(), _ptr(bias),
+                                            _ptr(residual), y.data_ptr(), _ptr(ws), B, ci, cout, H, W, _stream()),
+            "skp_conv3x3_f4r_pre_f32")
+    return y
+
+
+class ResnetInnerFn(torch.autograd.Function):
+
+    @staticmethod
+    def forward(ctx, h, w1, off, gamma, beta, groups: int, eps: float, w2, bias, residual):
+        h = _dev(h, "h")
+        B, _, H, W = h.shape
+        C, C2 = int(w1.shape[0]), int(w2.shape[0])
+        lib, dev = N.lib(), h.device
+        off_c = _dev(off.reshape(B, C), "off") if off is not None else None
+        residual = _dev(residual, "residual") if residual is not None else None
+        part, S = _conv3x3_parts(h, w1, False, C)
+        y1 = part.view(B, C, H, W) if S == 1 else torch.empty(B, C, H, W, device=dev, dtype=torch.float32)
+        mean = torch.empty(B, groups, device=dev, dtype=torch.float32)
+        rstd = torch.empty_like(mean)
+        raw2 = _tiles_ok(B, C, groups, H, W, C2)
+        tiles = _workspace("skp_conv3x3_f4r_tiles_workspace", B, C, H, W, device=dev) if raw2 else None
+        h2 = torch.empty(B, C, H, W, device=dev, dtype=torch.float32)
+        N.check(lib.skp_group_norm_fwd_parts_f32(part.data_ptr(), S, None if S == 1 else y1.data_ptr(), _ptr(off_c),
+                                                 gamma.data_ptr(), beta.data_ptr(), h2.data_ptr(), _ptr(tiles), mean.data_ptr(),
+                                                 rstd.data_ptr(), B, C, groups, H, W, float(eps), 1, _stream()),
+                "skp_group_norm_fwd_parts_f32")
+        if raw2:
+            out = _conv3x3_f4r_pre(tiles, w2, False, bias, residual, (B, C, H, W), C2)
+        else:
+            out = _conv3x3_run(h2, w2, False, bias, residual, C2)
+        ctx.save_for_backward(y1, off_c if off_c is not None else y1.new_empty(0), gamma, beta, mean, rstd)
+        ctx.w = (w1, w2)
+        ctx.meta = (groups, float(eps), off_c is not None)
+        return out
+
+    @staticmethod
+    def backward(ctx, dout):
+        dh = None
+        if ctx.needs_input_grad[0]:
+            y1, off_c, gamma, beta, mean, rstd = ctx.saved_tensors
+            groups, eps, has_off = ctx.meta
+            w1, w2 = ctx.w
+            dout = _dev(dout, "dout")
+            B, C, H, W = y1.shape
+            C1 = int(w1.shape[1])
+            dpart, S = _conv3x3_parts(dout, w2, True, C)
+            raw1 = _tiles_ok(B, C, groups, H, W, C1)
+            tiles = _workspace("skp_conv3x3_f4r_tiles_workspace", B, C, H, W, device=dout.device) if raw1 else None
+            dy1 = torch.empty_like(y1)
+            N.check(N.lib().skp_group_norm_bwd_parts_f32(y1.data_ptr(), off_c.data_ptr() if has_off else None, gamma.data_ptr(),
+                                                         beta.data_ptr(), dpart.data_ptr(), S, mean.data_ptr(), rstd.data_ptr(),
+                                                         dy1.data_ptr(), _ptr(tiles), B, C, groups, H, W, eps, 1, _stream()),
+                    "skp_group_norm_bwd_parts_f32")
+            if raw1:
+                dh = _conv3x3_f4r_pre(tiles, w1, True, None, None, (B, C, H, W), C1)
+            else:
+                dh = _conv3x3_run(dy1, w1, True, None, None, C1)
+        return dh, None, None, None, None, None, None, None, None, (dout if ctx.needs_input_grad[9] else None)
+
+
+def resnet_inner(h, w1, norm: torch.nn.GroupNorm, w2, off=None, bias=None, residual=None):
+    return ResnetInnerFn.apply(h, w1, off, norm.weight, norm.bias, norm.num_groups, norm.eps, w2, bias, residual)
+
+
 GN_FOLD = True
 
 
```

Measured after the change: 52.90 (median of 3 runs). No clear change (-0.7%).
